# RKlompUU/fhe-regex

Measured on AMD Instinct MI355X. Metric: TFHE gate-bootstraps/sec; end-to-end match time for /abc/ on 256-char content, higher is better.
Workload: dtype u64

## Files before the change

### fhe-regex_amd/csrc/device.h

```cpp
#pragma once
#include <cstdint>
#include <vector>

#include "common.h"
#include "owned.h"

namespace fr {

constexpr int MAX_OUT = 8;
enum : int32_t { JOB_MULTI = 0, JOB_DIRECT = 1, JOB_SIGN = 2, JOB_ACC = 3 };
struct DevGate {
    int32_t n_in;
    int32_t offset;
    int32_t in_slot[16];
    int32_t in_w[16];
    int32_t n_out;
    int32_t direct;
    int32_t out_slot[MAX_OUT];
    uint8_t lut[MAX_OUT][16];
};
static_assert(sizeof(DevGate) == 304, "DevGate layout");
constexpr int MAX_SELECTORS = 2 * (int)NEEDLE_MAX_CHARS;
FR_HD uint32_t acc_selector(const DevGate& g) {
    return (uint32_t)g.lut[0][0] | ((uint32_t)g.lut[0][1] << 8) | ((uint32_t)g.lut[0][2] << 16) |
           ((uint32_t)g.lut[0][3] << 24);
}
inline void set_acc_selector(DevGate& g, uint32_t q) {
    for (int i = 0; i < 4; ++i) g.lut[0][i] = (uint8_t)(q >> (8 * i));
}
int lut_w_norm2(const uint8_t* lut);

struct DeviceTimers {
    double br_ms = 0, ks_ms = 0;
    uint64_t br_launches = 0, br_gates = 0, lut_outputs = 0;
    double lat_br_ms = 0;
    uint64_t lat_launches = 0, lat_gates = 0;
    double pair_br_ms = 0;
    uint64_t pair_launches = 0, pair_gates = 0;
};

struct ClientKey;
struct RngKey;
class Device;
using Slots = gpu::SlotsOf<Device>;

struct DevNeedle {
    gpu::DevBuf<uint64_t> words;
    size_t m = 0;
    Device* dev = nullptr;
    DevNeedle() = default;
    DevNeedle(DevNeedle&&) = default;
    DevNeedle& operator=(DevNeedle&&) = delete;
    ~DevNeedle();
};

class Device {
  public:
    Device(const Params& p, int device);
    ~Device();
    Device(const Device&) = delete;
    Device& operator=(const Device&) = delete;

    const Params& params() const { return p_; }
    int device() const { return dev_; }

    void upload_keys(const std::vector<uint64_t>& ksk, const std::vector<uint64_t>& bsk);
    bool has_keys() const { return ksk_ && (p_.ring == FR_RING_FFT ? bool(d_fbsk_[0]) : bool(d_bsk_)); }
    void gen_server_key(const ClientKey& ck, const RngKey& key, const RngKey* mask_key = nullptr);
    void load_server_key_compact(const RngKey& mask_key, const uint8_t* bodies);
    const double* key_load_ms() const { return key_load_ms_; }
    void download_server_key(uint64_t* ksk, size_t ksk_len, uint64_t* bsk, size_t bsk_len);
    void gen_packing_key(const ClientKey& ck, const RngKey& mask_key, const RngKey& noise_key, bool compact = false);
    void upload_packing_key(const void* rows);
    void download_packing_key(uint64_t* rows);
    void load_packing_key_compact(const RngKey& mask_key, const uint8_t* planes);
    void download_packing_key_compact(uint8_t* planes);
    const double* pk_load_ms() const { return pk_load_ms_; }
    bool has_packing_key() const { return bool(pksk_); }
    void packing_limb_column(int col, uint64_t* out_host);
    void pack_bools(const DevGate* gates, size_t n, uint64_t* out_host);
    void pack_bools_compact(const DevGate* gates, size_t n, uint16_t* out_host );
    const double* pack_ms() const { return pack_ms_; }
    void encrypt_to_slots(const ClientKey& ck, const uint8_t* msgs, size_t count, const RngKey& key, uint64_t first_block,
                          const int* slots);

    Slots expand_to_slots(const RngKey& mask_key, uint64_t first_block, const uint8_t* bodies, size_t count);
    double expand_ms() const { return expand_ms_; }

    int alloc_slot();
    void free_slot(int s);
    void write_slots(const int* slots, size_t n, const uint64_t* host );
    void read_slot(int slot, uint64_t* host );
    void slots_to_device(const int* slots, size_t n, uint64_t* dst);
    void device_to_slots(const int* slots, size_t n, const uint64_t* src);
    void slots_to_device_async(const int* slots, size_t n, uint64_t* dst);
    void* stream() const { return cur().stream.get(); }
    void zero_slot(int slot);
    size_t arena_slots() const { return next_slot_; }
    size_t arena_free_slots() const { return free_slots_.size(); }

    void run_level(const DevGate* gates, size_t n);
    void run_level_resident(const DevGate* d_gates, const DevGate* host, size_t n, size_t n_refs = 0);
    gpu::DevBuf<DevGate> upload_gates(const DevGate* gates, size_t n, size_t n_refs = 0);
    void bind_content(const int* cmap, size_t n);
    DevNeedle upload_needle(const uint64_t* words, size_t m);
    void bind_selectors(const uint64_t* table, size_t count);
    void run_linear(const DevGate& g);
    void sync();

    void set_lanes(int n);
    int match_lanes() const { return (int)lanes_.size(); }
    void enter_lane(int i);
    void leave_lane();
    void set_profiling(int level) { profiling_ = level; }
    DeviceTimers& timers() { return timers_; }

    void keyswitch_host(const uint64_t* in, size_t count, uint64_t* out);
    void blind_rotate_host(const uint64_t* ks_in, const uint8_t* luts, size_t count, uint64_t* out);
    void blind_rotate_multi_host(const uint64_t* ks_in, const uint8_t* luts, int n_out, int direct, uint64_t* out);
    void blind_rotate_acc_host(const uint64_t* ks_in, const uint64_t* accs, size_t count, uint64_t* out);
    void ring_mul_host(const uint64_t* a, const uint64_t* b, size_t count, uint64_t* out);
    void bench_pbs(const std::vector<DevGate>& gates, int iters, double* br_ms, double* total_ms);

    std::string info() const;

  private:
    struct LaneState {
        gpu::Stream stream;
        gpu::DevBuf<uint64_t> ks;
        gpu::DevBuf<int8_t> dig;
        gpu::DevBuf<DevGate> pk_gates;
        gpu::DevBuf<int8_t> pk_dig;
        gpu::DevBuf<uint64_t> pk_g;
        gpu::DevBuf<uint16_t> pk_c16;
        gpu::DevBuf<double> kpre;
        gpu::StagingRing<int> cmap;
        size_t cmap_n = 0;
        const uint64_t* sel = nullptr;
        size_t sel_n = 0;
        gpu::Event done_ev;
        bool pending = false;
    };
    LaneState lane0_;
    std::vector<LaneState> lanes_;
    int lane_ = 0;
    LaneState& cur() { return lane_ ? lanes_[lane_ - 1] : lane0_; }
    const LaneState& cur() const { return lane_ ? lanes_[lane_ - 1] : lane0_; }
    bool lanes_pending_ = false;
    bool lanes_unsynced_ = false;
    gpu::Event main_ev_;
    std::vector<int> deferred_free_;
    hipStream_t cur_stream();
    void join_lanes();
    void sync_all();
    void ensure_arena(size_t slots);
    void ensure_ks(size_t n);
    void ensure_gates(size_t n);
    void validate_gates(const DevGate* gates, size_t n, size_t n_refs = 0) const;
    void launch_level(const DevGate* d_gates, const DevGate* host, size_t n);
    gpu::Event take_event();
    void resolve_timers();
    void ensure_digits(size_t rows);
    struct LimbKey {
        gpu::DevBuf<uint64_t> rows;
        gpu::DevBuf<int8_t> limbs;
        int KD = 0, ncols = 0, nlc = 0;
        explicit operator bool() const { return rows && limbs; }
        void alloc_rows(int kd, int nc) {
            limbs.reset();
            KD = kd, ncols = nc, nlc = ((nc * 8 + 127) / 128) * 128;
            rows.alloc((size_t)kd * nc);
        }
        void reset() { rows.reset(), limbs.reset(); }
    };
    void build_limbs(LimbKey& key);
    void drop_server_key() {
        ksk_.reset(), d_tbsk_.reset(), d_bsk_.reset(), d_fbsk_[0].reset(), d_fbsk_[1].reset();
        lane0_.kpre.reset();
        for (auto& l : lanes_) l.kpre.reset();
    }
    void drop_packing_key() { pksk_.reset(); }
    struct KsShape {
        int MR;
        size_t padded;
        int MC = 1, GZ = 1;
        bool lds = true;
    };
    KsShape ks_shape(size_t n) const {
        const int MR = n >= ks_mr4_min_ ? 4 : 1;
        return {MR, (n + 32 * MR - 1) / (32 * MR) * (32 * MR)};
    }
    template <int KSB, int KSL>
    void launch_ks_digits(const DevGate* d_gates, size_t n, size_t padded, int8_t* dig, uint64_t* out, int out_n,
                          int out_stride, hipEvent_t ev_start);
    void launch_limb_gemm(const int8_t* dig, const LimbKey& key, size_t n, const KsShape& sh, uint64_t* out,
                          int out_stride, hipEvent_t ev_stop);
    void launch_ks(const DevGate* d_gates, size_t n, uint64_t* d_ks, hipEvent_t ev_start = nullptr,
                   hipEvent_t ev_stop = nullptr);
    void launch_br(const DevGate* d_gates, const uint64_t* d_ks, size_t n, hipEvent_t ev_start = nullptr,
                   hipEvent_t ev_stop = nullptr, bool acc = false);
    size_t leading_selector_jobs(const DevGate* host, size_t n) const;
    void launch_jobs(const DevGate* d_gates, const DevGate* host, size_t n, bool acc);
    void run_br_jobs(const uint64_t* ks_in, std::vector<DevGate>& gates, uint64_t* out);
    void init_rns();
    void upload_rns_bsk(const std::vector<uint64_t>& bsk);
    void launch_br_rns(const DevGate* d_gates, const uint64_t* d_ks, size_t n, hipEvent_t ev_start, hipEvent_t ev_stop);
    void init_ks();
    void init_fft();
    void upload_fft_bsk(const std::vector<uint64_t>& bsk);
    void launch_br_fft(const DevGate* d_gates, const uint64_t* d_ks, size_t n, hipStream_t stream,
                       hipEvent_t ev_start = nullptr, hipEvent_t ev_stop = nullptr, bool acc = false);
    void build_fourier_bsk();
    double key_load_ms_[5] = {0, 0, 0, 0, 0};
    double pk_load_ms_[3] = {0, 0, 0};
    gpu::StagingRing<uint8_t> xstage_;
    double expand_ms_ = 0;
    void stage_slot_list(const int* slots, size_t n);
    gpu::DevBuf<int> d_slot_list_;

    Params p_;
    int dev_;
    int e_ = 8;
    int e_small_ = 8;
    size_t small_batch_ = 256;
    LimbKey ksk_;
    gpu::DevBuf<uint64_t> d_tbsk_;
    LimbKey pksk_;
    double pack_ms_[4] = {0, 0, 0, 0};
    void pack_launch(const DevGate* gates, size_t n, uint64_t* out_words, uint16_t* out_c16);
    int pk_split_ = 0;
    bool ks_mfma_ = true;
    size_t ks_mr4_min_ = 96;
    int ks_mc_ = 0;
    int ks_split_ = 0;
    int ks_xcd_ = 1;
    bool ks_dig16_ = true;
    bool ks_lds_ = true;
    gpu::DevBuf<uint32_t> d_bsk_;
    gpu::DevBuf<uint32_t> d_tw_;
    int fft_e_ = 4;
    size_t fft_small_ = 256;
    size_t fft_pair_ = SIZE_MAX;
    bool fft_dual_ = false;
    size_t fft_kpre_ = 32;
    gpu::DevBuf<double> d_fbsk_[2];
    static int fbsk_index(int E) { return E == 4 ? 0 : 1; }
    bool fbsk_needed(int E) const { return E == 4 || E == fft_e_; }
    gpu::DevBuf<double> d_ftw_;
    gpu::DevBuf<double> d_fqt_;
    gpu::DevBuf<uint16_t> d_fleaf_;
    gpu::DevBuf<uint64_t> d_arena_;
    std::vector<int> free_slots_;
    size_t next_slot_ = 0;
    gpu::StagingRing<DevGate> gates_;
    struct PendingTimer {
        gpu::Event ev[4];
        size_t gates, outs;
        bool lat, pair, ks;
        bool chain;
    };
    bool latency_shape(size_t n) const;
    bool pair_shape(size_t n) const;
    std::vector<PendingTimer> pending_;
    std::vector<gpu::Event> event_pool_;
    int profiling_ = 0;
    bool timer_chain_ = true;
    DeviceTimers timers_;
    gpu::Event ev_[4];
};

}
```

### fhe-regex_amd/csrc/device.hip

```cpp
#include <algorithm>
#include <cstdlib>
#include <cstring>
#include <sstream>

#include "device_impl.h"

namespace fr {

static bool supported(const Params& p) {
    if (p.ring == FR_RING_FFT) return (p.N == 2048 && p.k == 1) || (p.N == 1024 && p.k == 2);
    return (p.N == 2048 && p.k == 1) || (p.N == 1024 && p.k == 2) || (p.N == 1024 && p.k == 1);
}

namespace gpu {
void* dev_alloc(size_t bytes) {
    void* p = nullptr;
    HIP_CHECK(hipMalloc(&p, bytes));
    return p;
}
void dev_free(void* p) noexcept { (void)hipFree(p); }
void* pinned_alloc(size_t bytes) {
    void* p = nullptr;
    HIP_CHECK(hipHostMalloc(&p, bytes));
    return p;
}
void pinned_free(void* p) noexcept { (void)hipHostFree(p); }
hipEvent_t event_create(unsigned flags) {
    hipEvent_t e = nullptr;
    HIP_CHECK(hipEventCreateWithFlags(&e, flags));
    return e;
}
void event_destroy(hipEvent_t e) noexcept { (void)hipEventDestroy(e); }
hipStream_t stream_create() {
    hipStream_t s = nullptr;
    HIP_CHECK(hipStreamCreateWithFlags(&s, hipStreamNonBlocking));
    return s;
}
void stream_destroy(hipStream_t s) noexcept { (void)hipStreamDestroy(s); }

void StagingBytes::reserve(size_t bytes, size_t first, hipStream_t s) {
    if (bytes <= d_.size()) return;
    size_t cap = d_.size() ? d_.size() : first;
    while (cap < bytes) cap *= 2;
    HIP_CHECK(hipStreamSynchronize(s));
    d_.reset();
    for (auto& h : h_) h.reset();
    try {
        for (auto& e : ev_)
            if (!e) e = Event(hipEventDisableTiming);
        for (auto& h : h_) h.alloc(cap);
        d_.alloc(cap);
    } catch (...) {
        for (auto& h : h_) h.reset();
        throw;
    }
}
void* StagingBytes::acquire() {
    side_ ^= 1;
    HIP_CHECK(hipEventSynchronize(ev_[side_].get()));
    return h_[side_].get();
}
void StagingBytes::commit(size_t bytes, hipStream_t s) {
    HIP_CHECK(hipMemcpyAsync(d_.get(), h_[side_].get(), bytes, hipMemcpyHostToDevice, s));
    HIP_CHECK(hipEventRecord(ev_[side_].get(), s));
}
}

Device::Device(const Params& p, int device) : p_(p), dev_(device) {
    if (!supported(p)) throw Error(FR_ERR_INVALID, "device: unsupported (k, N)");
    if (p.ks_base_log != 3 || p.ks_level != 5 || p.pbs_base_log != 23 || p.pbs_level != 1)
        throw Error(FR_ERR_INVALID, "device: only KS 2^3x5 and PBS 2^23x1 are compiled");
    if (p.n > 1024) throw Error(FR_ERR_INVALID, "device: n > 1024");
    int count = 0;
    if (hipGetDeviceCount(&count) != hipSuccess || count <= device || device < 0)
        throw Error(FR_ERR_NO_DEVICE, "no usable HIP device " + std::to_string(device));
    HIP_CHECK(hipSetDevice(device));
    lane0_.stream.create();
    for (auto& e : ev_) e = gpu::Event(hipEventDefault);
    init_rns();
    init_ks();
    if (const char* ev = std::getenv("FR_TIMER_CHAIN")) timer_chain_ = std::atoi(ev) != 0;
    if (p.ring == FR_RING_FFT) init_fft();
    ensure_arena(1024);
    ensure_ks(1024);
    ensure_gates(1024);
}

Device::~Device() {
    (void)hipSetDevice(dev_);
    for (auto& l : lanes_) (void)hipStreamSynchronize(l.stream.get());
    if (lane0_.stream) (void)hipStreamSynchronize(lane0_.stream.get());
}

void Device::set_lanes(int n) {
    if (n < 1 || n > 8) throw Error(FR_ERR_INVALID, "lanes: 1..8");
    if (lane_ != 0) throw Error(FR_ERR_INVALID, "lanes: changed inside a lane");
    sync_all();
    const int extra = n >= 2 ? n : 0;
    while ((int)lanes_.size() > extra) lanes_.pop_back();
    if (!main_ev_ && extra) main_ev_ = gpu::Event(hipEventDisableTiming);
    while ((int)lanes_.size() < extra) {
        LaneState l;
        l.stream.create();
        l.done_ev = gpu::Event(hipEventDisableTiming);
        lanes_.push_back(std::move(l));
        enter_lane((int)lanes_.size());
        ensure_ks(1024);
        leave_lane();
    }
}
void Device::enter_lane(int i) {
    if (lane_ != 0) throw Error(FR_ERR_INVALID, "lanes: already inside a lane");
    if (i <= 0) return;
    if (i > (int)lanes_.size()) throw Error(FR_ERR_INVALID, "lanes: no such lane");
    HIP_CHECK(hipEventRecord(main_ev_.get(), lane0_.stream.get()));
    HIP_CHECK(hipStreamWaitEvent(lanes_[i - 1].stream.get(), main_ev_.get(), 0));
    lane_ = i;
}
void Device::leave_lane() {
    if (lane_ == 0) return;
    LaneState& l = cur();
    HIP_CHECK(hipEventRecord(l.done_ev.get(), l.stream.get()));
    l.pending = true;
    lanes_pending_ = true;
    lanes_unsynced_ = true;
    lane_ = 0;
}
void Device::join_lanes() {
    if (!lanes_pending_ || lane_ != 0) return;
    for (auto& l : lanes_)
        if (l.pending) {
            HIP_CHECK(hipStreamWaitEvent(lane0_.stream.get(), l.done_ev.get(), 0));
            l.pending = false;
        }
    lanes_pending_ = false;
}
hipStream_t Device::cur_stream() {
    if (lane_ == 0 && lanes_pending_) join_lanes();
    return cur().stream.get();
}
void Device::sync_all() {
    HIP_CHECK(hipStreamSynchronize(lane0_.stream.get()));
    for (auto& l : lanes_) HIP_CHECK(hipStreamSynchronize(l.stream.get()));
    if (lane_ == 0) {
        for (auto& l : lanes_) l.pending = false;
        lanes_pending_ = false;
    }
    lanes_unsynced_ = false;
    free_slots_.insert(free_slots_.end(), deferred_free_.begin(), deferred_free_.end());
    deferred_free_.clear();
}

std::string Device::info() const {
    hipDeviceProp_t prop;
    (void)hipGetDeviceProperties(&prop, dev_);
    std::ostringstream o;
    o << prop.name << " " << prop.gcnArchName << " CUs=" << prop.multiProcessorCount;
    if (p_.ring == FR_RING_FFT) o << " ring=fft E=" << fft_e_ << " latency<=" << fft_small_;
    else o << " ring=rns E=" << e_;
    return o.str();
}

void Device::ensure_arena(size_t slots) {
    const size_t stride = p_.slot_stride(), have = d_arena_.size() / stride;
    if (slots <= have) return;
    size_t cap = have ? have : 1024;
    while (cap < slots) cap *= 2;
    gpu::DevBuf<uint64_t> nb(stride * cap);
    if (d_arena_) {
        sync_all();
        HIP_CHECK(hipMemcpyAsync(nb.get(), d_arena_.get(), 8 * d_arena_.size(), hipMemcpyDeviceToDevice, STREAM));
        HIP_CHECK(hipStreamSynchronize(STREAM));
    }
    d_arena_ = std::move(nb);
}

void Device::ensure_ks(size_t n) {
    const size_t row = p_.ks_stride();
    if (n * row <= cur().ks.size()) return;
    HIP_CHECK(hipStreamSynchronize(STREAM));
    cur().ks.grow(n * row, 1024 * row);
}
void Device::ensure_gates(size_t n) { gates_.reserve(n, 1024, STREAM); }

int Device::alloc_slot() {
    if (!free_slots_.empty()) {
        int s = free_slots_.back();
        free_slots_.pop_back();
        return s;
    }
    ensure_arena(next_slot_ + 1);
    return (int)next_slot_++;
}
void Device::free_slot(int s) {
    if (s < 0) return;
    if (lanes_unsynced_ || lane_ != 0) {
        deferred_free_.push_back(s);
        if (deferred_free_.size() >= (size_t)1 << 16) sync_all();
    } else {
        free_slots_.push_back(s);
    }
}

__global__ void __launch_bounds__(256) k_slots_to_buf(const uint64_t* __restrict__ arena, int stride,
                                                      const int* __restrict__ slots, int len, uint64_t* __restrict__ buf) {
    const uint64_t* s = arena + (size_t)slots[blockIdx.x] * stride;
    uint64_t* d = buf + (size_t)blockIdx.x * len;
    for (int c = threadIdx.x; c < len; c += 256) d[c] = s[c];
}
__global__ void __launch_bounds__(256) k_buf_to_slots(const uint64_t* __restrict__ buf, int len,
                                                      const int* __restrict__ slots, int stride, uint64_t* __restrict__ arena) {
    const uint64_t* s = buf + (size_t)blockIdx.x * len;
    uint64_t* d = arena + (size_t)slots[blockIdx.x] * stride;
    for (int c = threadIdx.x; c < len; c += 256) d[c] = s[c];
}
struct SlotArgs {
    int s[16];
};
__global__ void __launch_bounds__(256) k_slots_to_buf_arg(const uint64_t* __restrict__ arena, int stride, SlotArgs sl,
                                                          int len, uint64_t* __restrict__ buf) {
    const uint64_t* s = arena + (size_t)sl.s[blockIdx.x] * stride;
    uint64_t* d = buf + (size_t)blockIdx.x * len;
    for (int c = threadIdx.x; c < len; c += 256) d[c] = s[c];
}
void Device::slots_to_device_async(const int* slots, size_t n, uint64_t* dst) {
    if (!n) return;
    if (n > 16) throw Error(FR_ERR_INVALID, "slots_to_device_async: at most 16 slots");
    SlotArgs a{};
    for (size_t i = 0; i < n; ++i) {
        if (slots[i] < 0 || (size_t)slots[i] >= next_slot_) throw Error(FR_ERR_INVALID, "slot list: slot out of range");
        a.s[i] = slots[i];
    }
    k_slots_to_buf_arg<<<(unsigned)n, 256, 0, STREAM>>>(d_arena_.get(), p_.slot_stride(), a, p_.lwe_len(), dst);
    HIP_CHECK(hipGetLastError());
}
void Device::stage_slot_list(const int* slots, size_t n) {
    for (size_t i = 0; i < n; ++i)
        if (slots[i] < 0 || (size_t)slots[i] >= next_slot_) throw Error(FR_ERR_INVALID, "slot list: slot out of range");
    if (n > d_slot_list_.size()) {
        HIP_CHECK(hipStreamSynchronize(STREAM));
        d_slot_list_.alloc(std::max<size_t>(n, 1024));
    }
    HIP_CHECK(hipMemcpyAsync(d_slot_list_.get(), slots, 4 * n, hipMemcpyHostToDevice, STREAM));
}
void Device::slots_to_device(const int* slots, size_t n, uint64_t* dst) {
    if (!n) return;
    stage_slot_list(slots, n);
    k_slots_to_buf<<<(unsigned)n, 256, 0, STREAM>>>(d_arena_.get(), p_.slot_stride(), d_slot_list_.get(), p_.lwe_len(), dst);
    HIP_CHECK(hipGetLastError());
    HIP_CHECK(hipStreamSynchronize(STREAM));
}
void Device::device_to_slots(const int* slots, size_t n, const uint64_t* src) {
    if (!n) return;
    stage_slot_list(slots, n);
    k_buf_to_slots<<<(unsigned)n, 256, 0, STREAM>>>(src, p_.lwe_len(), d_slot_list_.get(), p_.slot_stride(), d_arena_.get());
    HIP_CHECK(hipGetLastError());
    HIP_CHECK(hipStreamSynchronize(STREAM));
}

void Device::write_slots(const int* slots, size_t n, const uint64_t* host) {
    const int L = p_.lwe_len(), S = p_.slot_stride();
    for (size_t i = 0; i < n; ++i)
        HIP_CHECK(hipMemcpyAsync(d_arena_.get() + (size_t)slots[i] * S, host + i * L, 8 * (size_t)L, hipMemcpyHostToDevice, STREAM));
    HIP_CHECK(hipStreamSynchronize(STREAM));
}
void Device::read_slot(int slot, uint64_t* host) {
    HIP_CHECK(hipMemcpyAsync(host, d_arena_.get() + (size_t)slot * p_.slot_stride(), 8 * (size_t)p_.lwe_len(),
                             hipMemcpyDeviceToHost, STREAM));
    sync_all();
}
void Device::zero_slot(int slot) {
    HIP_CHECK(hipMemsetAsync(d_arena_.get() + (size_t)slot * p_.slot_stride(), 0, 8 * (size_t)p_.lwe_len(), STREAM));
}

void Device::upload_keys(const std::vector<uint64_t>& ksk, const std::vector<uint64_t>& bsk) {
    if (ksk.size() != (size_t)p_.big() * p_.ks_level * (p_.n + 1)) throw Error(FR_ERR_INVALID, "ksk size");
    if (bsk.size() != p_.bsk_len()) throw Error(FR_ERR_INVALID, "bsk size");
    Replacing key_guard([this] { drop_server_key(); });
    ksk_.alloc_rows(p_.big() * p_.ks_level, p_.n + 1);
    HIP_CHECK(hipMemcpy(ksk_.rows.get(), ksk.data(), 8 * ksk.size(), hipMemcpyHostToDevice));
    build_limbs(ksk_);
    if (p_.ring == FR_RING_FFT) upload_fft_bsk(bsk);
    else upload_rns_bsk(bsk);
    key_guard.dismiss();
}

bool Device::latency_shape(size_t n) const { return n <= (p_.ring == FR_RING_FFT ? fft_small_ : small_batch_); }
bool Device::pair_shape(size_t n) const { return p_.ring == FR_RING_FFT && !latency_shape(n) && n <= fft_pair_; }

void Device::launch_br(const DevGate* d_gates, const uint64_t* d_ks, size_t n, hipEvent_t ev_start, hipEvent_t ev_stop,
                       bool acc) {
    if (acc && p_.ring != FR_RING_FFT) throw Error(FR_ERR_INVALID, "private search: FFT ring only");
    if (p_.ring == FR_RING_FFT) launch_br_fft(d_gates, d_ks, n, cur().stream.get(), ev_start, ev_stop, acc);
    else launch_br_rns(d_gates, d_ks, n, ev_start, ev_stop);
}

void Device::validate_gates(const DevGate* gates, size_t n, size_t n_refs) const {
    for (size_t i = 0; i < n; ++i) {
        const DevGate& g = gates[i];
        if (g.n_in < 0 || g.n_in > 16 || g.n_out < 1 || g.n_out > MAX_OUT || g.direct < 0 || g.direct > JOB_ACC ||
            (g.direct && g.n_out != 1))
            throw Error(FR_ERR_INVALID, "device gate: bad descriptor");
        if (g.direct == JOB_ACC) {
            if (p_.ring != FR_RING_FFT) throw Error(FR_ERR_INVALID, "private search: FFT ring only");
            if (acc_selector(g) >= (uint32_t)MAX_SELECTORS) throw Error(FR_ERR_INVALID, "device gate: bad selector index");
        }
        for (int f = 0; f < g.n_out; ++f)
            if (g.out_slot[f] < 0 || (size_t)g.out_slot[f] >= next_slot_) throw Error(FR_ERR_INVALID, "device gate: bad output slot");
        for (int q = 0; q < g.n_in; ++q) {
            const int s = g.in_slot[q];
            if (s >= 0 ? (size_t)s >= next_slot_ : (size_t)(-1 - (int64_t)s) >= n_refs)
                throw Error(FR_ERR_INVALID, "device gate: bad input slot");
        }
    }
}

void Device::bind_content(const int* cmap, size_t n) {
    for (size_t i = 0; i < n; ++i)
        if (cmap[i] < -1 || (cmap[i] >= 0 && (size_t)cmap[i] >= next_slot_))
            throw Error(FR_ERR_INVALID, "content map: slot out of range");
    LaneState& l = cur();
    const size_t bound = l.cmap_n;
    l.cmap_n = 0;
    if (!n) return;
    const hipStream_t s = STREAM;
    l.cmap.reserve(n, 4096, s);
    if (n != bound || std::memcmp(l.cmap.last(), cmap, 4 * n) != 0) {
        std::memcpy(l.cmap.acquire(), cmap, 4 * n);
        l.cmap.commit(n, s);
    }
    l.cmap_n = n;
}

DevNeedle::~DevNeedle() {
    if (!words || !dev) return;
    try {
        dev->sync();
    } catch (...) {
    }
}

DevNeedle Device::upload_needle(const uint64_t* words, size_t m) {
    if (p_.ring != FR_RING_FFT) throw Error(FR_ERR_INVALID, "private search: FFT ring only");
    if (!words || m < 1 || 2 * m > (size_t)MAX_SELECTORS) throw Error(FR_ERR_INVALID, "needle: 1 <= m <= 64");
    DevNeedle nd;
    nd.dev = this;
    nd.m = m;
    nd.words.alloc(2 * m * (size_t)(p_.k + 1) * p_.N);
    HIP_CHECK(hipMemcpy(nd.words.get(), words, 8 * nd.words.size(), hipMemcpyHostToDevice));
    return nd;
}

void Device::bind_selectors(const uint64_t* table, size_t count) {
    if (table && p_.ring != FR_RING_FFT) throw Error(FR_ERR_INVALID, "private search: FFT ring only");
    cur().sel = table;
    cur().sel_n = table ? count : 0;
}

size_t Device::leading_selector_jobs(const DevGate* host, size_t n) const {
    if (!n || host[0].direct != JOB_ACC) return 0;
    size_t a = 0;
    while (a < n && host[a].direct == JOB_ACC) ++a;
    for (size_t i = 0; i < n; ++i) {
        if (host[i].direct != JOB_ACC) continue;
        if (i >= a) throw Error(FR_ERR_INVALID, "selector jobs must lead their level");
        if ((size_t)acc_selector(host[i]) >= cur().sel_n)
            throw Error(FR_ERR_INVALID, "selector job: index past the selector table bound");
    }
    return a;
}

void Device::run_level(const DevGate* gates, size_t n) {
    if (!n) return;
    if (!has_keys()) throw Error(FR_ERR_NO_KEY, "server key not uploaded");
    if (lane_ != 0) throw Error(FR_ERR_INVALID, "staged gate batches run on lane 0 only");
    validate_gates(gates, n);
    ensure_ks(n);
    ensure_gates(n);
    std::memcpy(gates_.acquire(), gates, sizeof(DevGate) * n);
    gates_.commit(n, STREAM);
    launch_level(gates_.device(), gates, n);
}

void Device::run_level_resident(const DevGate* d_gates, const DevGate* host, size_t n, size_t n_refs) {
    if (!n) return;
    if (!has_keys()) throw Error(FR_ERR_NO_KEY, "server key not uploaded");
    if (n_refs > cur().cmap_n) throw Error(FR_ERR_INVALID, "template plan: content map not bound");
    ensure_ks(n);
    launch_level(d_gates, host, n);
}

gpu::DevBuf<DevGate> Device::upload_gates(const DevGate* gates, size_t n, size_t n_refs) {
    validate_gates(gates, n, n_refs);
    gpu::DevBuf<DevGate> d(std::max<size_t>(n, 1));
    HIP_CHECK(hipMemcpy(d.get(), gates, sizeof(DevGate) * n, hipMemcpyHostToDevice));
    return d;
}

void Device::launch_level(const DevGate* d_gates, const DevGate* host, size_t n) {
    const size_t a = leading_selector_jobs(host, n);
    if (a) launch_jobs(d_gates, host, a, true);
    if (n > a) launch_jobs(d_gates + a, host + a, n - a, false);
}

void Device::launch_jobs(const DevGate* d_gates, const DevGate* host, size_t n, bool acc) {
    PendingTimer t{};
    if (profiling_)
        for (auto& e : t.ev) e = take_event();
    t.chain = profiling_ == 1 && timer_chain_;
    uint64_t* d_ks = cur().ks.get();
    if (profiling_ >= 2) launch_ks(d_gates, n, d_ks, t.ev[0].get(), t.ev[1].get());
    else launch_ks(d_gates, n, d_ks, nullptr, t.chain ? t.ev[1].get() : nullptr);
    launch_br(d_gates, d_ks, n, t.chain ? nullptr : t.ev[2].get(), t.ev[3].get(), acc);
    HIP_CHECK(hipGetLastError());
    if (profiling_) {
        t.gates = n;
        t.lat = latency_shape(n);
        t.pair = pair_shape(n) && (!fft_dual_ || acc);
        t.ks = profiling_ >= 2;
        t.outs = 0;
        for (size_t i = 0; i < n; ++i) t.outs += host[i].n_out;
        pending_.push_back(std::move(t));
    }
}

gpu::Event Device::take_event() {
    if (!event_pool_.empty()) {
        gpu::Event e = std::move(event_pool_.back());
        event_pool_.pop_back();
        return e;
    }
    for (unsigned fl : {(unsigned)hipEventReleaseToDevice, (unsigned)hipEventDisableSystemFence})
        try {
            return gpu::Event(fl);
        } catch (const Error&) {
            (void)hipGetLastError();
        }
    return gpu::Event(hipEventDefault);
}
void Device::resolve_timers() {
    for (auto& t : pending_) {
        float ks = 0, br = 0;
        if (t.ks) HIP_CHECK(hipEventElapsedTime(&ks, t.ev[0].get(), t.ev[1].get()));
        HIP_CHECK(hipEventElapsedTime(&br, t.ev[t.chain ? 1 : 2].get(), t.ev[3].get()));
        timers_.ks_ms += ks;
        timers_.br_ms += br;
        timers_.br_launches += 1;
        timers_.br_gates += t.gates;
        timers_.lut_outputs += t.outs;
        if (t.lat) {
            timers_.lat_br_ms += br;
            timers_.lat_launches += 1;
            timers_.lat_gates += t.gates;
        }
        if (t.pair) {
            timers_.pair_br_ms += br;
            timers_.pair_launches += 1;
            timers_.pair_gates += t.gates;
        }
        for (auto& e : t.ev)
            if (e) event_pool_.push_back(std::move(e));
    }
    pending_.clear();
}

void Device::sync() {
    sync_all();
    resolve_timers();
}

void Device::keyswitch_host(const uint64_t* in, size_t count, uint64_t* out) {
    if (!has_keys()) throw Error(FR_ERR_NO_KEY, "server key not uploaded");
    HIP_CHECK(hipStreamSynchronize(STREAM));
    Slots slots(*this, count);
    std::vector<DevGate> gates(count);
    write_slots(slots.data(), count, in);
    for (size_t i = 0; i < count; ++i) {
        std::memset(&gates[i], 0, sizeof(DevGate));
        gates[i].n_in = 1;
        gates[i].in_slot[0] = slots[i];
        gates[i].in_w[0] = 1;
        gates[i].n_out = 1;
        gates[i].direct = JOB_DIRECT;
        gates[i].out_slot[0] = slots[i];
    }
    ensure_ks(count);
    ensure_gates(count);
    uint64_t* d_ks = cur().ks.get();
    HIP_CHECK(hipMemcpy(gates_.device(), gates.data(), sizeof(DevGate) * count, hipMemcpyHostToDevice));
    launch_ks(gates_.device(), count, d_ks);
    HIP_CHECK(hipStreamSynchronize(STREAM));
    const int ks = p_.ks_stride();
    for (size_t i = 0; i < count; ++i)
        HIP_CHECK(hipMemcpy(out + i * (p_.n + 1), d_ks + i * ks, 8 * (size_t)(p_.n + 1), hipMemcpyDeviceToHost));
}

static DevGate br_job(const uint8_t* luts, int n_out, int direct) {
    DevGate g;
    std::memset(&g, 0, sizeof g);
    g.n_out = n_out;
    g.direct = direct;
    std::memcpy(g.lut, luts, 16 * (size_t)n_out);
    return g;
}

void Device::run_br_jobs(const uint64_t* ks_in, std::vector<DevGate>& gates, uint64_t* out) {
    if (!has_keys()) throw Error(FR_ERR_NO_KEY, "server key not uploaded");
    HIP_CHECK(hipStreamSynchronize(STREAM));
    const size_t count = gates.size();
    ensure_ks(count);
    ensure_gates(count);
    uint64_t* d_ks = cur().ks.get();
    const int ks = p_.ks_stride();
    for (size_t i = 0; i < count; ++i)
        HIP_CHECK(hipMemcpy(d_ks + i * ks, ks_in + i * (p_.n + 1), 8 * (size_t)(p_.n + 1), hipMemcpyHostToDevice));
    size_t n_out = 0;
    for (auto& g : gates) n_out += (size_t)g.n_out;
    Slots slots(*this, n_out);
    n_out = 0;
    for (auto& g : gates)
        for (int f = 0; f < g.n_out; ++f) g.out_slot[f] = slots[n_out++];
    HIP_CHECK(hipMemcpy(gates_.device(), gates.data(), sizeof(DevGate) * count, hipMemcpyHostToDevice));
    const size_t a = leading_selector_jobs(gates.data(), count);
    if (a && a != count) throw Error(FR_ERR_INVALID, "a launch is all selector jobs or none");
    PendingTimer t{};
    if (profiling_) {
        t.ev[2] = take_event(), t.ev[3] = take_event();
        t.gates = count, t.outs = n_out;
        t.lat = latency_shape(count);
        t.pair = pair_shape(count) && (!fft_dual_ || a != 0);
    }
    launch_br(gates_.device(), d_ks, count, t.ev[2].get(), t.ev[3].get(), a != 0);
    if (profiling_) {
        pending_.push_back(std::move(t));
        sync();
    } else {
        HIP_CHECK(hipStreamSynchronize(STREAM));
    }
    for (size_t i = 0; i < slots.size(); ++i) read_slot(slots[i], out + i * p_.lwe_len());
}

void Device::blind_rotate_acc_host(const uint64_t* ks_in, const uint64_t* accs, size_t count, uint64_t* out) {
    if (p_.ring != FR_RING_FFT) throw Error(FR_ERR_INVALID, "private search: FFT ring only");
    if (!has_keys()) throw Error(FR_ERR_NO_KEY, "server key not uploaded");
    if (lane_ != 0) throw Error(FR_ERR_INVALID, "parity hooks run on lane 0 only");
    if (!count) return;
    const size_t W = (size_t)(p_.k + 1) * p_.N;
    gpu::DevBuf<uint64_t> table(count * W);
    HIP_CHECK(hipMemcpy(table.get(), accs, 8 * count * W, hipMemcpyHostToDevice));
    std::vector<DevGate> gates(count);
    for (size_t i = 0; i < count; ++i) {
        std::memset(&gates[i], 0, sizeof(DevGate));
        gates[i].n_out = 1;
        gates[i].direct = JOB_ACC;
        set_acc_selector(gates[i], (uint32_t)i);
    }
    const uint64_t* prev = cur().sel;
    const size_t prev_n = cur().sel_n;
    bind_selectors(table.get(), count);
    try {
        run_br_jobs(ks_in, gates, out);
    } catch (...) {
        (void)hipStreamSynchronize(cur().stream.get());
        bind_selectors(prev, prev_n);
        throw;
    }
    bind_selectors(prev, prev_n);
}

void Device::blind_rotate_host(const uint64_t* ks_in, const uint8_t* luts, size_t count, uint64_t* out) {
    std::vector<DevGate> gates(count);
    for (size_t i = 0; i < count; ++i) gates[i] = br_job(luts + 16 * i, 1, JOB_DIRECT);
    run_br_jobs(ks_in, gates, out);
}

void Device::blind_rotate_multi_host(const uint64_t* ks_in, const uint8_t* luts, int n_out, int direct,
                                     uint64_t* out) {
    if (!has_keys()) throw Error(FR_ERR_NO_KEY, "server key not uploaded");
    if (n_out < 1 || n_out > MAX_OUT || direct < 0 || direct > 2 || (direct && n_out != 1))
        throw Error(FR_ERR_INVALID, "bad n_out");
    std::vector<DevGate> gates{br_job(luts, n_out, direct)};
    run_br_jobs(ks_in, gates, out);
}

int lut_w_norm2(const uint8_t* lut) {
    int s = 0;
    for (int m = 1; m < 16; ++m) s += ((int)lut[m] - lut[m - 1]) * ((int)lut[m] - lut[m - 1]);
    s += ((int)lut[0] + lut[15]) * ((int)lut[0] + lut[15]);
    return s;
}

void Device::bench_pbs(const std::vector<DevGate>& gates, int iters, double* br_ms, double* total_ms) {
    const size_t n = gates.size();
    ensure_ks(n);
    ensure_gates(n);
    sync();
    std::memcpy(gates_.acquire(), gates.data(), sizeof(DevGate) * n);
    gates_.commit(n, STREAM);
    const DevGate* d_gates = gates_.device();
    uint64_t* d_ks = cur().ks.get();
    float br_sum = 0;
    HIP_CHECK(hipEventRecord(ev_[3].get(), STREAM));
    for (int it = 0; it < iters; ++it) {
        launch_ks(d_gates, n, d_ks);
        HIP_CHECK(hipEventRecord(ev_[1].get(), STREAM));
        launch_br(d_gates, d_ks, n);
        HIP_CHECK(hipEventRecord(ev_[2].get(), STREAM));
        HIP_CHECK(hipEventSynchronize(ev_[2].get()));
        float br = 0;
        HIP_CHECK(hipEventElapsedTime(&br, ev_[1].get(), ev_[2].get()));
        br_sum += br;
    }
    HIP_CHECK(hipEventRecord(ev_[0].get(), STREAM));
    HIP_CHECK(hipEventSynchronize(ev_[0].get()));
    float tot = 0;
    HIP_CHECK(hipEventElapsedTime(&tot, ev_[3].get(), ev_[0].get()));
    *br_ms = br_sum;
    *total_ms = tot;
}

}
```

### fhe-regex_amd/csrc/fft_br.hip

```cpp
#include <hip/hip_ext.h>
#include <hip/hip_runtime.h>

#include <cstring>

#include "device_impl.h"
#include "fft.h"
#include "geo.h"

namespace fr {

template <int M, int E>
using FGeo = NttGeo<M, E, 3, fft_layout_variant(ilog2c(M), ilog2c(E))>;
template <int M, int E>
constexpr int FV = fft_layout_variant(ilog2c(M), ilog2c(E));

__device__ __forceinline__ void cfwd(double2& x, double2& y, double2 c) { fft::fwd_bf(x.x, x.y, y.x, y.y, c.x, c.y); }
__device__ __forceinline__ void cinv(double2& u, double2& v, double2 c) { fft::inv_bf(u.x, u.y, v.x, v.y, c.x, c.y); }

template <int M, int E>
constexpr bool fradix4() {
    return E == 4 && FGeo<M, E>::LOG % 2 == 0;
}
template <int M, int E>
struct FTwr {
    static constexpr int COUNT = fradix4<M, E>() ? FGeo<M, E>::NPH * 3 : FGeo<M, E>::LOG * (E / 2);
    double2 v[COUNT];
};
__device__ __forceinline__ double2 fmul_i(double2 c) { return make_double2(-c.y, c.x); }
__device__ __forceinline__ void cinv_r4(double2 (&x)[4], double2 c, double2 ca, double2 cc) {
    fft::inv_r4(x[0].x, x[0].y, x[1].x, x[1].y, x[2].x, x[2].y, x[3].x, x[3].y, c.x, c.y, ca.x, ca.y, cc.x, cc.y);
}
template <class G, int E, int p, bool REV, class F>
__device__ __forceinline__ void for_butterflies(F&& fn) {
#pragma unroll
    for (int i = 0; i < G::s_end(p) - G::s_begin(p); ++i) {
        const int s = REV ? G::s_end(p) - 1 - i : G::s_begin(p) + i;
        const int dm = 1 << (G::LOG - 1 - s - G::lo(p));
#pragma unroll
        for (int m = 0; m < E; ++m) {
            if (m & dm) continue;
            fn(s, m, dm);
        }
    }
}
template <class G, int p>
__device__ __forceinline__ double2 ftw_at(const double2* tw, int b, int s, int m) {
    return (tw + (b >> (G::LOG - s)))[(1 << s) + (G::template moff<p>(m) >> (G::LOG - s))];
}
template <int M, int E, int p>
__device__ __forceinline__ void ftw_r4(const double2* tw, int tl, double2& c, double2& ca) {
    using G = FGeo<M, E>;
    constexpr int s0 = G::s_begin(p), s1 = s0 + 1;
    const int b = G::template base<p>(tl);
    c = ftw_at<G, p>(tw, b, s0, 0);
    ca = ftw_at<G, p>(tw, b, s1, 0);
}

template <int M, int E, int p>
__device__ __forceinline__ void ffwd_phase(double2 (&x)[E], const double2* tw, int tl) {
    using G = FGeo<M, E>;
    const int b = G::template base<p>(tl);
    for_butterflies<G, E, p, false>([&](int s, int m, int dm) { cfwd(x[m], x[m + dm], ftw_at<G, p>(tw, b, s, m)); });
}
template <int M, int E, int p>
__device__ __forceinline__ void finv_phase(double2 (&x)[E], const double2* tw, int tl) {
    using G = FGeo<M, E>;
    const int b = G::template base<p>(tl);
    for_butterflies<G, E, p, true>([&](int s, int m, int dm) { cinv(x[m], x[m + dm], ftw_at<G, p>(tw, b, s, m)); });
}
template <int M, int E, int p>
__device__ __forceinline__ void finv_phase_lds(double2 (&x)[E], const double2* tw, const double2* twc, int tl) {
    if constexpr (fradix4<M, E>()) {
        using G = FGeo<M, E>;
        double2 c, ca;
        ftw_r4<M, E, p>(tw, tl, c, ca);
        const double2 cc = ftw_at<G, p>(twc, G::template base<p>(tl), G::s_begin(p), 0);
        cinv_r4(x, c, ca, cc);
    } else {
        finv_phase<M, E, p>(x, tw, tl);
    }
}

#ifndef FR_LAT_LOAD1
#define FR_LAT_LOAD1 2
#endif
#ifndef FR_LAT_LOAD2
#define FR_LAT_LOAD2 3
#endif
#ifndef FR_LAT_PF
#define FR_LAT_PF 2
#endif
#ifndef FR_LAT_PF2
#define FR_LAT_PF2 2
#endif
#ifndef FR_PAIR_LOAD
#define FR_PAIR_LOAD 2
#endif
#ifndef FR_PAIR_PF
#define FR_PAIR_PF 1
#endif
#ifndef FR_PAIR_LOAD2
#define FR_PAIR_LOAD2 4
#endif
#ifndef FR_PAIR_CC
#define FR_PAIR_CC 1
#endif
#ifndef FR_LAT_TWR
#define FR_LAT_TWR 1
#endif

template <int M, int E, int p>
constexpr bool ftw_wave_uniform() {
    using G = FGeo<M, E>;
    for (int w = 0; w * 64 < G::T; ++w)
        for (int s = G::s_begin(p); s < G::s_end(p); ++s) {
            const int ref = geo_base(G::LOG, G::e, p, w * 64, FV<M, E>) >> (G::LOG - s);
            for (int l = 1; l < 64; ++l)
                if ((geo_base(G::LOG, G::e, p, w * 64 + l, FV<M, E>) >> (G::LOG - s)) != ref) return false;
        }
    return true;
}
__device__ __forceinline__ double2 fwave_uniform(double2 v) {
    const unsigned long long a = (unsigned long long)__double_as_longlong(v.x);
    const unsigned long long b = (unsigned long long)__double_as_longlong(v.y);
    const unsigned a0 = __builtin_amdgcn_readfirstlane((unsigned)a), a1 = __builtin_amdgcn_readfirstlane((unsigned)(a >> 32));
    const unsigned b0 = __builtin_amdgcn_readfirstlane((unsigned)b), b1 = __builtin_amdgcn_readfirstlane((unsigned)(b >> 32));
    return make_double2(__longlong_as_double((long long)(((unsigned long long)a1 << 32) | a0)),
                        __longlong_as_double((long long)(((unsigned long long)b1 << 32) | b0)));
}
#ifndef FR_TW_SGPR_PAIR
#define FR_TW_SGPR_PAIR 1
#endif

template <int M, int E>
constexpr int ftw_index(int s, int m) {
    const int d = FGeo<M, E>::LOG - 1 - s - FGeo<M, E>::lo(s / FGeo<M, E>::e);
    return s * (E / 2) + ((m >> (d + 1)) << d) + (m & ((1 << d) - 1));
}
template <int M, int E, int p, bool UNI = false>
__device__ __forceinline__ void ftw_load_phase(FTwr<M, E>& twr, const double2* tw, int tl) {
    using G = FGeo<M, E>;
    if constexpr (fradix4<M, E>()) {
        double2 c, ca, cc;
        ftw_r4<M, E, p>(tw, tl, c, ca);
        fft::cmul(c.x, c.y, ca.x, ca.y, cc.x, cc.y);
        if constexpr (UNI && ftw_wave_uniform<M, E, p>()) {
            c = fwave_uniform(c);
            ca = fwave_uniform(ca);
            cc = fwave_uniform(cc);
        }
        twr.v[3 * p] = c, twr.v[3 * p + 1] = ca, twr.v[3 * p + 2] = cc;
        if constexpr (p + 1 < G::NPH) ftw_load_phase<M, E, p + 1, UNI>(twr, tw, tl);
        return;
    }
    const int b = G::template base<p>(tl);
    for_butterflies<G, E, p, false>([&](int s, int m, int) { twr.v[ftw_index<M, E>(s, m)] = ftw_at<G, p>(tw, b, s, m); });
    if constexpr (p + 1 < G::NPH) ftw_load_phase<M, E, p + 1, UNI>(twr, tw, tl);
}
template <int M, int E, int p>
__device__ __forceinline__ void ffwd_phase_r(double2 (&x)[E], const FTwr<M, E>& twr) {
    using G = FGeo<M, E>;
    if constexpr (fradix4<M, E>()) {
        const double2 c = twr.v[3 * p], ca = twr.v[3 * p + 1];
        cfwd(x[0], x[2], c);
        cfwd(x[1], x[3], c);
        cfwd(x[0], x[1], ca);
        cfwd(x[2], x[3], fmul_i(ca));
        return;
    }
    for_butterflies<G, E, p, false>([&](int s, int m, int dm) { cfwd(x[m], x[m + dm], twr.v[ftw_index<M, E>(s, m)]); });
}
template <int M, int E, int p>
__device__ __forceinline__ void finv_phase_r(double2 (&x)[E], const FTwr<M, E>& twr) {
    using G = FGeo<M, E>;
    if constexpr (fradix4<M, E>()) {
        cinv_r4(x, twr.v[3 * p], twr.v[3 * p + 1], twr.v[3 * p + 2]);
        return;
    }
    for_butterflies<G, E, p, true>([&](int s, int m, int dm) { cinv(x[m], x[m + dm], twr.v[ftw_index<M, E>(s, m)]); });
}

template <int M, int E, int PF, int PT>
constexpr int fperm_lane_bit(int j) {
    using G = FGeo<M, E>;
    const int out = G::lo(PF) + j, in = G::lo(PT) + j;
    int kb = -1, kc = -1;
    for (int b = 0; b < 6; ++b) {
        if (G::lane_bit(PT, b) == out) kb = b;
        if (G::lane_bit(PF, b) == in) kc = b;
    }
    return kb == kc ? kb : -1;
}
template <int M, int E, int PF, int PT>
constexpr bool fperm_ok() {
    using G = FGeo<M, E>;
    if (PF == PT || (PF - PT != 1 && PT - PF != 1)) return false;
    for (int j = 0; j < G::e; ++j) {
        const int k = fperm_lane_bit<M, E, PF, PT>(j);
        if (k != 4 && k != 5) return false;
    }
    for (int b = 0; b < 8; ++b) {
        bool swapped = false;
        for (int j = 0; j < G::e; ++j) swapped |= fperm_lane_bit<M, E, PF, PT>(j) == b;
        if (!swapped && G::lane_bit(PF, b) != G::lane_bit(PT, b)) return false;
    }
    return true;
}
template <int K>
__device__ __forceinline__ void fperm_swap(double& a, double& b) {
    static_assert(K == 4 || K == 5, "permlane swaps serve lane bits 4 and 5");
    const unsigned long long ua = (unsigned long long)__double_as_longlong(a);
    const unsigned long long ub = (unsigned long long)__double_as_longlong(b);
    unsigned lo0 = (unsigned)ua, hi0 = (unsigned)(ua >> 32), lo1 = (unsigned)ub, hi1 = (unsigned)(ub >> 32);
    if constexpr (K == 4) {
        const auto l = __builtin_amdgcn_permlane16_swap(lo0, lo1, false, false);
        const auto h = __builtin_amdgcn_permlane16_swap(hi0, hi1, false, false);
        lo0 = l[0], lo1 = l[1], hi0 = h[0], hi1 = h[1];
    } else {
        const auto l = __builtin_amdgcn_permlane32_swap(lo0, lo1, false, false);
        const auto h = __builtin_amdgcn_permlane32_swap(hi0, hi1, false, false);
        lo0 = l[0], lo1 = l[1], hi0 = h[0], hi1 = h[1];
    }
    a = __longlong_as_double((long long)(((unsigned long long)hi0 << 32) | lo0));
    b = __longlong_as_double((long long)(((unsigned long long)hi1 << 32) | lo1));
}
template <int M, int E, int PF, int PT, int j = 0>
__device__ __forceinline__ void fperm_exchange(double2 (&x)[E]) {
    constexpr int K = fperm_lane_bit<M, E, PF, PT>(j);
#pragma unroll
    for (int m = 0; m < E; ++m) {
        if (m & (1 << j)) continue;
        fperm_swap<K>(x[m].x, x[m | (1 << j)].x);
        fperm_swap<K>(x[m].y, x[m | (1 << j)].y);
    }
    if constexpr (j + 1 < FGeo<M, E>::e) fperm_exchange<M, E, PF, PT, j + 1>(x);
}

#ifndef FR_XKEEP
#define FR_XKEEP 1
#endif
template <int M, int E, int PF, int PT>
constexpr bool fxkeep_ok() {
    using G = FGeo<M, E>;
    if (!FR_XKEEP || (1 << (6 + G::e)) > G::T || PF == PT) return false;
    for (int b = 0; (1 << b) < G::T; ++b) {
        if (b >= 6 && b < 6 + G::e) {
            if (G::lane_bit(PF, b) != G::lo(PT) + (b - 6) || G::lane_bit(PT, b) != G::lo(PF) + (b - 6)) return false;
        } else if (G::lane_bit(PF, b) != G::lane_bit(PT, b)) {
            return false;
        }
    }
    return true;
}
template <int M, int E, int PF, int PT, bool PRE, bool XK, int B, int BS>
__device__ __forceinline__ void fexchange(double2 (&x)[B][E], double2* row, int tl) {
    using G = FGeo<M, E>;
    if constexpr (fperm_ok<M, E, PF, PT>()) {
        static_assert(!PRE, "register exchanges replace only exchanges without a pre-barrier");
#pragma unroll
        for (int b = 0; b < B; ++b) fperm_exchange<M, E, PF, PT>(x[b]);
    } else {
        constexpr int X = PF < PT ? PF : PT;
        double2* rf = row + G::template at<X>(G::template base<PF>(tl));
        double2* rt = row + G::template at<X>(G::template base<PT>(tl));
        if constexpr (PRE) __syncthreads();
        if constexpr (XK && fxkeep_ok<M, E, PF, PT>()) {
            const int q = __builtin_amdgcn_readfirstlane((tl >> 6) & (E - 1));
#pragma unroll
            for (int b = 0; b < B; ++b)
#pragma unroll
                for (int m = 0; m < E; ++m)
                    if (m != q) rf[b * BS + G::template at<X>(G::template moff<PF>(m))] = x[b][m];
            __syncthreads();
#pragma unroll
            for (int b = 0; b < B; ++b)
#pragma unroll
                for (int m = 0; m < E; ++m)
                    if (m != q) x[b][m] = rt[b * BS + G::template at<X>(G::template moff<PT>(m))];
            return;
        }
#pragma unroll
        for (int b = 0; b < B; ++b)
#pragma unroll
            for (int m = 0; m < E; ++m) rf[b * BS + G::template at<X>(G::template moff<PF>(m))] = x[b][m];
        if constexpr (G::template wave_local<PF, PT>() && G::wave_top(PF)) wave_sync();
        else __syncthreads();
#pragma unroll
        for (int b = 0; b < B; ++b)
#pragma unroll
            for (int m = 0; m < E; ++m) x[b][m] = rt[b * BS + G::template at<X>(G::template moff<PT>(m))];
    }
}
template <int M, int E, int X = 0>
constexpr bool fexchanges_conflict_free() {
    using G = FGeo<M, E>;
    if constexpr (X + 1 >= G::NPH) return true;
    else
        return ((fperm_ok<M, E, X, X + 1>() && X != G::XL) || G::template b128_exchange_ok<X>()) &&
               fexchanges_conflict_free<M, E, X + 1>();
}
template <int M, int E, int p, bool NOPRE, bool TWR, int B, int BS, bool CARRY = false, class Hook>
__device__ __forceinline__ void fforward_from(double2 (&x)[B][E], double2* row, const FTwr<M, TWR ? E : 2>& twr,
                                              const double2* tw, int tl, Hook&& hook) {
#pragma unroll
    for (int b = 0; b < B; ++b) {
        if constexpr (TWR) ffwd_phase_r<M, E, p>(x[b], twr);
        else ffwd_phase<M, E, p>(x[b], tw, tl);
    }
    hook(std::integral_constant<int, p>{});
    if constexpr (p + 1 < FGeo<M, E>::NPH) {
        constexpr bool pre = !NOPRE && (FGeo<M, E>::template fwd_pre<p>() || CARRY), reg = fperm_ok<M, E, p, p + 1>();
        fexchange<M, E, p, p + 1, reg ? false : pre, !NOPRE, B, BS>(x, row, tl);
        fforward_from<M, E, p + 1, NOPRE, TWR, B, BS, reg && pre>(x, row, twr, tw, tl, hook);
    }
}
template <int M, int E, int p, bool NOPRE, bool TWR, int B, int BS, bool CARRY = false>
__device__ __forceinline__ void finverse_from(double2 (&x)[B][E], double2* row, const FTwr<M, TWR ? E : 2>& twr,
                                              const double2* tw, const double2* twc, int tl) {
    if constexpr (TWR && B > 1 && fradix4<M, E>() && FR_PAIR_CC) {
        const double2 c = twr.v[3 * p], ca = twr.v[3 * p + 1];
        double2 cc;
        fft::cmul(c.x, c.y, ca.x, ca.y, cc.x, cc.y);
#pragma unroll
        for (int b = 0; b < B; ++b) cinv_r4(x[b], c, ca, cc);
    } else {
#pragma unroll
        for (int b = 0; b < B; ++b) {
            if constexpr (TWR) finv_phase_r<M, E, p>(x[b], twr);
            else finv_phase_lds<M, E, p>(x[b], tw, twc, tl);
        }
    }
    if constexpr (p > 0) {
        constexpr bool pre = !NOPRE && (FGeo<M, E>::template inv_pre<p>() || CARRY), reg = fperm_ok<M, E, p, p - 1>();
        fexchange<M, E, p, p - 1, reg ? false : pre, !NOPRE, B, BS>(x, row, tl);
        finverse_from<M, E, p - 1, NOPRE, TWR, B, BS, reg && pre>(x, row, twr, tw, twc, tl);
    }
}

template <int N, int K, int E>
constexpr int fbr_threads() {
    return (K + 1) * (N / 2 / E);
}
__device__ __forceinline__ int psi_slot(int k) { return k ^ ((k >> 6) & 15) ^ ((k >> 5) & 1); }

__device__ __forceinline__ void slot_factor(double br, double bi, uint32_t e, uint32_t sm, double& cr, double& ci) {
    const uint32_t q = (e * sm) & 3u;
    const bool swap = (sm & 1u) && (e & 1u);
    const double ar = swap ? -bi : br, ai = swap ? br : bi;
    const long long sg = (long long)((q >> 1) & 1u) << 63;
    cr = __longlong_as_double(__double_as_longlong(ar) ^ sg);
    ci = __longlong_as_double(__double_as_longlong(ai) ^ sg);
}
template <int N, bool PSIQ>
__device__ __forceinline__ void key_psi_base(const double2* psi, uint32_t e, uint32_t Lb, double& br, double& bi) {
    const uint32_t k = __umul24(e, Lb) & (2 * N - 1);
    if constexpr (!PSIQ) {
        const double2 c = psi[psi_slot((int)k)];
        br = c.x;
        bi = c.y;
    } else {
        const double2 q = psi[psi_slot((int)(k & (N / 2 - 1)))];
        fft::psi_quadrant(q.x, q.y, k >> (ilog2c(N) - 1), br, bi);
    }
}
template <int K, int NB, class KeyAt>
__device__ __forceinline__ void key_products(const double (&bre)[2][NB], const double (&bim)[2][NB], int mb, uint32_t ei,
                                             uint32_t ej, uint32_t sm, KeyAt&& key, double& kor, double& koi,
                                             double (&kxr)[K], double (&kxi)[K]) {
    double cr[3], ci[3];
#pragma unroll
    for (int h = 1; h < 3; ++h)
        slot_factor(bre[h - 1][mb], bim[h - 1][mb], h == 1 ? ei : ej, sm, cr[h], ci[h]);
    fft::cmul(cr[1], ci[1], cr[2], ci[2], cr[0], ci[0]);
#pragma unroll
    for (int gg = 0; gg < 3; ++gg) {
        const double c1r = cr[gg] - 1.0, c1i = ci[gg];
        const double2 Bo = key(gg, 0);
        if (gg == 0) fft::cmul(Bo.x, Bo.y, c1r, c1i, kor, koi);
        else fft::cmac(Bo.x, Bo.y, c1r, c1i, kor, koi);
#pragma unroll
        for (int q = 0; q < K; ++q) {
            const double2 Bx = key(gg, 1 + q);
            if (gg == 0) fft::cmul(Bx.x, Bx.y, c1r, c1i, kxr[q], kxi[q]);
            else fft::cmac(Bx.x, Bx.y, c1r, c1i, kxr[q], kxi[q]);
        }
    }
}
template <int K, bool LAT>
constexpr bool fbr_twr() {
    return LAT && K == 1 && FR_LAT_TWR;
}
template <int N, int K, int E, bool LAT>
constexpr int fbr_twc_entries() {
    return fradix4<N / 2, E>() && !fbr_twr<K, LAT>() ? N / 4 : 0;
}
template <int N, int K, int E, bool LAT, int B = 1, bool KP = false>
constexpr size_t fbr_smem_bytes() {
    return 16 * ((LAT ? 2 : 1) * B * (K + 1) * (size_t)FGeo<N / 2, E>::NP + (B == 1 ? (size_t)N / 2 : 0) +
                 (KP ? 0 : LAT && B == 1 ? 2 * (size_t)N : (size_t)N / 2) + (size_t)fbr_twc_entries<N, K, E, LAT>()) +
           B * (16 * MAX_OUT + 2 * 1026) + (B == 1 ? 4 * 17 * MAX_OUT : 0) + 2 * 514;
}
template <int K, int E>
constexpr int fbr_tp_groups() {
    return K == 1 ? 2 : (E == 8 ? 3 : 2);
}
template <int N, int K, int E, bool LAT>
constexpr int fbr_min_waves() {
    if (LAT) return 2;
    if (K == 1) return E == 4 ? 4 : 2;
    return E == 4 ? 3 : 2;
}
typedef unsigned int fr_v4u __attribute__((ext_vector_type(4)));
__device__ __forceinline__ __amdgpu_buffer_rsrc_t bsk_rsrc(const double2* bsk) {
    return __builtin_amdgcn_make_buffer_rsrc((void*)bsk, 0, 0x7fffffff, 0x00020000);
}
__device__ __forceinline__ double2 bsk_load(__amdgpu_buffer_rsrc_t r, uint32_t lane_off, uint32_t uoff) {
    const fr_v4u v = __builtin_amdgcn_raw_buffer_load_b128(r, (int)lane_off, (int)uoff, 0);
    double2 d;
    __builtin_memcpy(&d, &v, 16);
    return d;
}

template <int K>
__device__ __forceinline__ int other_row(int P, int q) {
    return q < P ? q : q + 1;
}
template <int M, int T, int K>
__device__ __forceinline__ void load_slot(double2 (&B)[3][K + 1], __amdgpu_buffer_rsrc_t rs, uint32_t sbase, int P,
                                          int m, uint32_t lane_off) {
    constexpr uint32_t GG = (uint32_t)(K + 1) * (K + 1) * M;
#pragma unroll
    for (int gg = 0; gg < 3; ++gg) {
        B[gg][0] = bsk_load(rs, lane_off, sbase + 16u * (gg * GG + (uint32_t)(P * (K + 1) + P) * M + (uint32_t)m * T));
#pragma unroll
        for (int q = 0; q < K; ++q)
            B[gg][1 + q] = bsk_load(
                rs, lane_off, sbase + 16u * (gg * GG + (uint32_t)(other_row<K>(P, q) * (K + 1) + P) * M + (uint32_t)m * T));
    }
}

template <int N>
__device__ __forceinline__ uint64_t test_poly(int t, bool direct, const uint8_t* lut0) {
    constexpr int box = N / 16, half = box / 2;
    if (!direct) return 1ULL << (DELTA_LOG - 1);
    const int mm = (t + half) / box;
    return mm < 16 ? (uint64_t)lut0[mm] << DELTA_LOG : (uint64_t)0 - ((uint64_t)lut0[0] << DELTA_LOG);
}
template <int N>
__device__ __forceinline__ uint64_t w_step64(const uint64_t* row, const uint32_t* terms, int nt, int j) {
    uint64_t acc = 0;
    for (int t = 0; t < nt; ++t) {
        const uint32_t tm = terms[t];
        int src = j - (int)(tm & 0xFFFF);
        int64_t d = (int64_t)(tm >> 16) - 128;
        if (src < 0) {
            src += N;
            d = -d;
        }
        acc += (uint64_t)d * row[src];
    }
    return acc;
}

template <int M, int E>
__device__ __forceinline__ void fbr_publish(uint64_t* arow, const double (&alo)[E], const double (&ahi)[E], int tl) {
#pragma unroll
    for (int m = 0; m < E; ++m) {
        const int j = FGeo<M, E>::template idx<0>(tl, m);
        arow[j] = fft::torus_of_acc(alo[m]);
        arow[j + M] = fft::torus_of_acc(ahi[m]);
    }
}
template <int N>
__device__ __forceinline__ void fbr_terms(int tid, int n_out, int kind, const uint8_t* lut, uint32_t* wterms, int* wcnt) {
    if (tid < n_out && kind == JOB_MULTI) wcnt[tid] = lut_terms<N>(lut + 16 * tid, wterms + 16 * tid);
}
template <int N, int K, int NT>
__device__ __forceinline__ void fbr_outputs(int tid, const uint64_t* ab, const DevGate& gate, int n_out, int kind,
                                            const uint32_t* wterms, const int* wcnt, uint64_t* arena, int slot_stride) {
    constexpr int big = K * N;
    if (kind != JOB_MULTI) {
        uint64_t* out = arena + (size_t)gate.out_slot[0] * slot_stride;
        const uint64_t post = kind == JOB_SIGN ? (1ULL << (DELTA_LOG - 1)) : 0;
        for (int c = tid; c <= big; c += NT) {
            const ExtractIdx x = extract_index<N, K>(c);
            const uint64_t v = ab[x.pp * N + x.j];
            out[c] = (x.neg ? (uint64_t)0 - v : v) + (c == big ? post : 0);
        }
        return;
    }
    for (int f = 0; f < n_out; ++f) {
        const uint32_t* tf = wterms + 16 * f;
        const int nt = wcnt[f];
        uint64_t* out = arena + (size_t)gate.out_slot[f] * slot_stride;
        for (int c = tid; c <= big; c += NT) {
            const ExtractIdx x = extract_index<N, K>(c);
            const uint64_t v = w_step64<N>(ab + x.pp * N, tf, nt, x.j);
            out[c] = x.neg ? (uint64_t)0 - v : v;
        }
    }
}

template <int N, int K>
constexpr uint32_t kpre_step_bytes() {
    return 16u * (uint32_t)((K + 1) * (K + 1) * (N / 2));
}

template <int N, int K, int E, bool LAT, int B, bool KP, bool ACC = false>
__device__ __forceinline__ void fbr_rotate(const uint64_t* ks, int ks_stride, int n, const DevGate* gates, int n_gates,
                                           const double2* bsk, const double2* tw_g, const double2* psi_g,
                                           const uint16_t* leaf_g, uint64_t* arena, int slot_stride, const double2* kpre,
                                           const uint64_t* sel = nullptr) {
    constexpr int M = N / 2;
    static_assert(!KP || (LAT && B == 1 && K == 1 && E == 4), "key products: the k = 1 latency shape");
    static_assert(!(ACC && KP), "selector launches never take the key-products path");
    using G = FGeo<M, E>;
    static_assert(fexchanges_conflict_free<M, E>(), "LDS maps must make every exchange conflict-free");
    static_assert(G::base_matches_geo(), "base<p> must be the index map the LDS-map proofs reason about");
    static_assert(G::key_slot_matches_idx(), "the Fourier key's lane layout is the last-phase layout");
    static_assert(!LAT || E == 4, "the latency shape holds a step's GGSW values in registers: E = 4");
    static_assert(B == 1 || (B == 2 && LAT && K == 1 && E == 4), "pair shape: the k = 1 latency geometry");
    constexpr int NB = E >= 4 ? E / 4 : 1;
    constexpr int T = M / E, NT = (K + 1) * T, LAST = G::NPH - 1, XL = G::XL;
    constexpr int LOG2N2 = G::LOG + 2;
    constexpr bool TWR = fbr_twr<K, LAT>();
    constexpr int BS = (K + 1) * G::NP;
    constexpr bool PSIQ = !LAT || B > 1;
    extern __shared__ __attribute__((aligned(16))) double2 fsm[];
    double2* xbuf = fsm;
    double2* ibuf = LAT ? xbuf + B * BS : xbuf;
    double2* tw = xbuf + (LAT ? 2 : 1) * B * BS;
    constexpr int NPSI = KP ? 0 : PSIQ ? N / 2 : 2 * N;
    double2* psi = tw + (B == 1 ? M : 0);
    double2* twc = psi + NPSI;
    constexpr int NTWC = fbr_twc_entries<N, K, E, LAT>();
    uint8_t* lut = (uint8_t*)(twc + NTWC);
    uint16_t* abar = (uint16_t*)(lut + B * 16 * MAX_OUT);
    uint32_t* wterms = B == 1 ? (uint32_t*)(abar + 1026) : (uint32_t*)ibuf;
    int* wcnt = (int*)(wterms + B * 16 * MAX_OUT);
    uint16_t* nxt = B == 1 ? (uint16_t*)(wcnt + MAX_OUT) : abar + B * 1026;

    const int tid = threadIdx.x;
    const int P = __builtin_amdgcn_readfirstlane(tid / T), tl = tid % T;
    int gb[B];
    bool has[B];
    const uint64_t* in[B];
    int n_out[B], kind[B];
#pragma unroll
    for (int b = 0; b < B; ++b) {
        const int gi = B * (int)blockIdx.x + b;
        has[b] = gi < n_gates;
        gb[b] = has[b] ? gi : B * (int)blockIdx.x;
        in[b] = ks + (size_t)gb[b] * ks_stride;
        n_out[b] = gates[gb[b]].n_out;
        kind[b] = gates[gb[b]].direct;
    }
    if constexpr (B == 1)
        for (int i = tid; i < M; i += NT) tw[i] = tw_g[i];
    for (int i = tid; i < NPSI; i += NT) psi[psi_slot(i)] = psi_g[i];
    for (int i = 1 + tid; i < NTWC; i += NT) {
        const int s0 = 31 - __builtin_clz((unsigned)i), b = i - (1 << s0);
        if (s0 & 1) continue;
        const double2 c = tw_g[i], ca = tw_g[(2 << s0) + 2 * b];
        fft::cmul(c.x, c.y, ca.x, ca.y, twc[i].x, twc[i].y);
    }
    uint32_t bbar[B];
#pragma unroll
    for (int b = 0; b < B; ++b) {
        uint8_t* lb = lut + b * 16 * MAX_OUT;
        uint16_t* ab = abar + b * 1026;
        for (int i = tid; i < 16 * n_out[b]; i += NT) lb[i] = gates[gb[b]].lut[i / 16][i % 16];
        for (int i = tid; i < n; i += NT) ab[i] = (uint16_t)mod_switch(in[b][i], LOG2N2);
        if (tid == 0) ab[n] = 0;
        bbar[b] = mod_switch(in[b][n], LOG2N2);
    }
    uint32_t Lb[NB];
#pragma unroll
    for (int bb = 0; bb < NB; ++bb)
        Lb[bb] = (1u + 4u * (__brev((uint32_t)G::template idx<LAST>(tl, 4 * bb)) >> (32 - G::LOG))) & (uint32_t)(M - 1);
    __syncthreads();

    double alo[B][E], ahi[B][E];
#pragma unroll
    for (int b = 0; b < B; ++b) {
        if constexpr (ACC) {
            const uint64_t* A = sel + ((size_t)acc_selector(gates[gb[b]]) * (K + 1) + P) * N;
#pragma unroll
            for (int m = 0; m < E; ++m) {
                const int j = G::template idx<0>(tl, m);
                uint64_t v[2];
#pragma unroll
                for (int h = 0; h < 2; ++h) {
                    const int s = (j + h * M + (int)bbar[b]) & (2 * N - 1);
                    const uint64_t tv = A[s & (N - 1)];
                    v[h] = s < N ? tv : (uint64_t)0 - tv;
                }
                alo[b][m] = fft::acc_of_torus(v[0]);
                ahi[b][m] = fft::acc_of_torus(v[1]);
            }
            continue;
        }
        const bool direct = kind[b] == JOB_DIRECT;
#pragma unroll
        for (int m = 0; m < E; ++m) {
            const int j = G::template idx<0>(tl, m);
            uint64_t v[2];
#pragma unroll
            for (int h = 0; h < 2; ++h) {
                const int s = (j + h * M + (int)bbar[b]) & (2 * N - 1);
                const uint64_t tv = test_poly<N>(s & (N - 1), direct, lut + b * 16 * MAX_OUT);
                v[h] = s < N ? tv : (uint64_t)0 - tv;
            }
            alo[b][m] = P == K ? fft::acc_of_torus(v[0]) : 0.0;
            ahi[b][m] = P == K ? fft::acc_of_torus(v[1]) : 0.0;
        }
    }

    double2* row = xbuf + P * G::NP;
    double2* irow = ibuf + P * G::NP;
    const int bl = G::template base<LAST>(tl);
    double2* row_bl = row + G::template at<XL>(bl);
    const double2* orow_bl[K];
#pragma unroll
    for (int q = 0; q < K; ++q) orow_bl[q] = xbuf + other_row<K>(P, q) * G::NP + G::template at<XL>(bl);
    constexpr uint32_t GG = (uint32_t)(K + 1) * (K + 1) * M;
    const __amdgpu_buffer_rsrc_t rs = bsk_rsrc(bsk);
    const uint32_t lane_off = 16u * (uint32_t)tl;
    const int steps = (n + 1) / 2;
    double2 gv[3][K + 1][LAT && !KP ? E : 1];
    double2 kv[K + 1][KP ? E : 1];
    FTwr<M, TWR ? E : 2> twr;
    if constexpr (TWR) ftw_load_phase<M, E, 0, B == 1 ? false : FR_TW_SGPR_PAIR>(twr, B == 1 ? tw : tw_g, tl);
#ifdef FR_BR_TIMING
    uint64_t tseg[6] = {0, 0, 0, 0, 0, 0};
    uint64_t tlast = __builtin_amdgcn_s_memtime();
    const uint64_t tstart = tlast;
#endif
    auto load_ggsw = [&](int gg, int tt) {
        if constexpr (!KP) {
            const uint32_t sb = (uint32_t)__builtin_amdgcn_readfirstlane(tt) * (3u * GG * 16u);
#pragma unroll
            for (int m = 0; m < E; ++m) {
                gv[gg][0][m] =
                    bsk_load(rs, lane_off, sb + 16u * (gg * GG + (uint32_t)(P * (K + 1) + P) * M + (uint32_t)m * T));
#pragma unroll
                for (int q = 0; q < K; ++q)
                    gv[gg][1 + q][m] = bsk_load(
                        rs, lane_off,
                        sb + 16u * (gg * GG + (uint32_t)(other_row<K>(P, q) * (K + 1) + P) * M + (uint32_t)m * T));
            }
        }
    };
    const __amdgpu_buffer_rsrc_t rk =
        bsk_rsrc(KP ? kpre + (size_t)blockIdx.x * ((size_t)((n + 1) / 2) * (kpre_step_bytes<N, K>() / 16)) : bsk);
    auto load_kp = [&](int tt) {
        if constexpr (KP) {
            const uint32_t sb = (uint32_t)__builtin_amdgcn_readfirstlane(tt) * kpre_step_bytes<N, K>();
#pragma unroll
            for (int r = 0; r <= K; ++r)
#pragma unroll
                for (int m = 0; m < E; ++m)
                    kv[r][m] = bsk_load(rk, lane_off, sb + 16u * (uint32_t)(((P * (K + 1) + r) * E + m) * T));
        }
    };
    constexpr int NPF = KP ? 0 : LAT ? (B > 1 ? FR_PAIR_PF : K == 1 ? FR_LAT_PF : FR_LAT_PF2) : 0;
    constexpr bool LATPF = NPF > 0;
    auto idle = [&](int t) {
        uint32_t z = 0;
#pragma unroll
        for (int b = 0; b < B; ++b) z |= abar[b * 1026 + 2 * t] | abar[b * 1026 + 2 * t + 1];
        return z == 0;
    };
    if constexpr (LATPF || KP) {
        for (int t = tid; t <= steps; t += NT) {
            int tt = t;
            while (tt < steps && idle(tt)) ++tt;
            nxt[t] = (uint16_t)tt;
        }
        __syncthreads();
        const int t0 = __builtin_amdgcn_readfirstlane((int)nxt[0]);
        for (int gg = 0; gg < NPF; ++gg) load_ggsw(gg, t0 < steps ? t0 : 0);
        load_kp(t0 < steps ? t0 : 0);
    }
    for (int t = 0; t < steps; ++t) {
        if (idle(t)) continue;
        BR_STAMP(0);
        const uint32_t sbase = (uint32_t)__builtin_amdgcn_readfirstlane(t) * (3u * GG * 16u);
        constexpr int G_TOP = !LAT || KP || B > 1 ? 3 : (NPF < 2 || K == 1) ? NPF : 3;
        constexpr int G_L1 = !LAT || KP ? 3 : B > 1 ? NPF : G_TOP + 1 < 3 ? G_TOP + 1 : 3;
        constexpr int G_L2 = !LAT || KP ? 3 : B > 1 ? (NPF + 1 < 3 ? NPF + 1 : 3) : G_TOP == 3 ? NPF : G_TOP + 2 < 3 ? G_TOP + 2 : 3;
        constexpr int PH_L1 = B > 1 ? FR_PAIR_LOAD : FR_LAT_LOAD1;
        constexpr int PH_L2 = B > 1 ? FR_PAIR_LOAD2 : FR_LAT_LOAD2;
        static_assert(G_L1 >= 3 || PH_L1 < G::NPH, "FR_PAIR_LOAD / FR_LAT_LOAD1 past the last forward phase");
        static_assert(G_L2 >= 3 || PH_L2 < G::NPH, "FR_PAIR_LOAD2 / FR_LAT_LOAD2 past the last forward phase");
        if constexpr (G_TOP < 3) {
            __builtin_amdgcn_sched_barrier(0);
            load_ggsw(G_TOP, t);
            __builtin_amdgcn_sched_barrier(0);
        }
        uint32_t ei[B], ej[B];
#pragma unroll
        for (int b = 0; b < B; ++b) {
            ei[b] = __builtin_amdgcn_readfirstlane((uint32_t)abar[b * 1026 + 2 * t]);
            ej[b] = __builtin_amdgcn_readfirstlane((uint32_t)abar[b * 1026 + 2 * t + 1]);
        }
        double bre[B][2][NB], bim[B][2][NB];
        auto psi_factors = [&]() {
#pragma unroll
            for (int b = 0; b < B; ++b)
#pragma unroll
                for (int h = 0; h < 2; ++h)
#pragma unroll
                    for (int bb = 0; bb < NB; ++bb)
                        key_psi_base<N, PSIQ>(psi, h == 0 ? ei[b] : ej[b], Lb[bb], bre[b][h][bb], bim[b][h][bb]);
        };
        if constexpr (LAT && B == 1 && !KP) psi_factors();
        double2 x[B][E];
#pragma unroll
        for (int b = 0; b < B; ++b)
#pragma unroll
            for (int m = 0; m < E; ++m)
                x[b][m] = make_double2(fft::acc_digit<23>(alo[b][m]), fft::acc_digit<23>(ahi[b][m]));
        BR_STAMP(1);
        fforward_from<M, E, 0, LAT, TWR, B, BS>(x, row, twr, tw, tl, [&](auto ph) {
            if constexpr (LAT) {
                constexpr int p = decltype(ph)::value;
                if constexpr (p == PH_L1 && G_L1 < 3) {
                    __builtin_amdgcn_sched_barrier(0);
                    load_ggsw(G_L1, t);
                    __builtin_amdgcn_sched_barrier(0);
                }
                if constexpr (p == PH_L2 && G_L2 < 3) {
                    __builtin_amdgcn_sched_barrier(0);
                    load_ggsw(G_L2, t);
                    __builtin_amdgcn_sched_barrier(0);
                }
            }
        });
        BR_STAMP(2);
#pragma unroll
        for (int b = 0; b < B; ++b)
#pragma unroll
            for (int m = 0; m < E; ++m) row_bl[b * BS + G::template at<XL>(G::template moff<LAST>(m))] = x[b][m];
        constexpr bool AHEAD = !LAT && E == 8;
        constexpr bool PRE0 = !LAT;
        double2 Bc[3][K + 1];
        if constexpr (PRE0) load_slot<M, T, K>(Bc, rs, sbase, P, 0, lane_off);
        __syncthreads();
        if constexpr (!LAT || B > 1) psi_factors();
#pragma unroll
        for (int m = 0; m < E; ++m) {
            double2 Bn[3][K + 1];
            if constexpr (AHEAD) {
                if (m + 1 < E) load_slot<M, T, K>(Bn, rs, sbase, P, m + 1, lane_off);
                __builtin_amdgcn_sched_barrier(0);
            } else if constexpr (!LAT) {
                if (!PRE0 || m > 0) load_slot<M, T, K>(Bc, rs, sbase, P, m, lane_off);
            }
#pragma unroll
            for (int b = 0; b < B; ++b) {
                const double2 own = x[b][m];
                double2 oth[K];
#pragma unroll
                for (int q = 0; q < K; ++q) oth[q] = orow_bl[q][b * BS + G::template at<XL>(G::template moff<LAST>(m))];
                double kor, koi, kxr[K], kxi[K];
                if constexpr (KP) {
                    kor = kv[0][m].x, koi = kv[0][m].y;
#pragma unroll
                    for (int q = 0; q < K; ++q) kxr[q] = kv[1 + q][m].x, kxi[q] = kv[1 + q][m].y;
                } else {
                    const uint32_t sm = ((m & 1) << 1) | ((m >> 1) & 1);
                    auto key_at = [&](int gg, int r) __attribute__((always_inline)) {
                        return LAT ? gv[gg][r][LAT ? m : 0] : Bc[gg][r];
                    };
                    key_products<K>(bre[b], bim[b], m >> 2, ei[b], ej[b], sm, key_at, kor, koi, kxr, kxi);
                }
                double zr, zi;
                fft::cmul(own.x, own.y, kor, koi, zr, zi);
#pragma unroll
                for (int q = 0; q < K; ++q) fft::cmac(oth[q].x, oth[q].y, kxr[q], kxi[q], zr, zi);
                x[b][m] = make_double2(zr, zi);
            }
            if constexpr (!LAT) {
                __builtin_amdgcn_sched_barrier(0);
            }
            if constexpr (AHEAD) {
#pragma unroll
                for (int gg = 0; gg < 3; ++gg)
#pragma unroll
                    for (int r = 0; r <= K; ++r) Bc[gg][r] = Bn[gg][r];
            }
        }
        if constexpr (LATPF || KP) {
            const int tn = __builtin_amdgcn_readfirstlane((int)nxt[t + 1]);
            __builtin_amdgcn_sched_barrier(0);
            for (int gg = 0; gg < NPF; ++gg) load_ggsw(gg, tn < steps ? tn : t);
            load_kp(tn < steps ? tn : t);
            __builtin_amdgcn_sched_barrier(0);
        }
        BR_STAMP(3);
        finverse_from<M, E, LAST, LAT, TWR, B, BS>(x, irow, twr, tw, twc, tl);
        BR_STAMP(4);
#pragma unroll
        for (int b = 0; b < B; ++b)
#pragma unroll
            for (int m = 0; m < E; ++m) {
                alo[b][m] = fft::acc_reduce<23>(alo[b][m] + x[b][m].x);
                ahi[b][m] = fft::acc_reduce<23>(ahi[b][m] + x[b][m].y);
            }
        BR_STAMP(5);
    }
#ifdef FR_BR_TIMING
    if (blockIdx.x == 0 && tid == 0)
        printf("FBR_TIMING E=%d LAT=%d steps=%d total=%lu digits=%lu fwd=%lu mac=%lu inv=%lu acc=%lu top=%lu\n", E, (int)LAT,
               steps, (unsigned long)(__builtin_amdgcn_s_memtime() - tstart), (unsigned long)tseg[1],
               (unsigned long)tseg[2], (unsigned long)tseg[3], (unsigned long)tseg[4], (unsigned long)tseg[5],
               (unsigned long)tseg[0]);
#endif

    __syncthreads();
    uint64_t* accs = (uint64_t*)xbuf;
    static_assert(B == 1 || 8 * B * (K + 1) * N <= 16 * B * BS, "pair shape: u64 rows inside the forward rows");
#pragma unroll
    for (int b = 0; b < B; ++b) {
        fbr_publish<M, E>(accs + (b * (K + 1) + P) * N, alo[b], ahi[b], tl);
        fbr_terms<N>(tid, n_out[b], kind[b], lut + b * 16 * MAX_OUT, wterms + b * 16 * MAX_OUT, wcnt + b * MAX_OUT);
    }
    __syncthreads();
#pragma unroll
    for (int b = 0; b < B; ++b)
        if (has[b])
            fbr_outputs<N, K, NT>(tid, accs + b * (K + 1) * N, gates[gb[b]], n_out[b], kind[b], wterms + b * 16 * MAX_OUT,
                                  wcnt + b * MAX_OUT, arena, slot_stride);
}

template <int N, int K, int E, bool LAT, int B = 1>
__global__ void __launch_bounds__((fbr_threads<N, K, E>()), (fbr_min_waves<N, K, E, LAT>()))
k_blind_rotate_fft(const uint64_t* __restrict__ ks, int ks_stride, int n, const DevGate* __restrict__ gates,
                   int n_gates, const double2* __restrict__ bsk, const double2* __restrict__ tw_g,
                   const double2* __restrict__ psi_g, const uint16_t* __restrict__ leaf_g, uint64_t* __restrict__ arena,
                   int slot_stride) {
    fbr_rotate<N, K, E, LAT, B, false>(ks, ks_stride, n, gates, n_gates, bsk, tw_g, psi_g, leaf_g, arena, slot_stride,
                                       nullptr);
}
template <int N, int K, int E, bool LAT, int B = 1>
__global__ void __launch_bounds__((fbr_threads<N, K, E>()), (fbr_min_waves<N, K, E, LAT>()))
k_blind_rotate_fft_kp(const uint64_t* __restrict__ ks, int ks_stride, int n, const DevGate* __restrict__ gates,
                      int n_gates, const double2* __restrict__ tw_g, uint64_t* __restrict__ arena, int slot_stride,
                      const double2* __restrict__ kpre) {
    fbr_rotate<N, K, E, LAT, B, true>(ks, ks_stride, n, gates, n_gates, nullptr, tw_g, nullptr, nullptr, arena,
                                      slot_stride, kpre);
}

template <int N, int K, int E, bool LAT, int B = 1>
__global__ void __launch_bounds__((fbr_threads<N, K, E>()), (fbr_min_waves<N, K, E, LAT>()))
k_blind_rotate_fft_acc(const uint64_t* __restrict__ ks, int ks_stride, int n, const DevGate* __restrict__ gates,
                       int n_gates, const double2* __restrict__ bsk, const double2* __restrict__ tw_g,
                       const double2* __restrict__ psi_g, const uint16_t* __restrict__ leaf_g,
                       uint64_t* __restrict__ arena, int slot_stride, const uint64_t* __restrict__ sel) {
    fbr_rotate<N, K, E, LAT, B, false, true>(ks, ks_stride, n, gates, n_gates, bsk, tw_g, psi_g, leaf_g, arena,
                                             slot_stride, nullptr, sel);
}

template <int N>
__global__ void __launch_bounds__(N / 8)
k_key_products(const uint64_t* __restrict__ ks, int ks_stride, int n, int n_gates, const double2* __restrict__ bsk,
               const double2* __restrict__ psi_g, double2* __restrict__ kpre) {
    constexpr int K = 1, E = 4, M = N / 2, T = M / E;
    using G = FGeo<M, E>;
    static_assert(G::key_slot_matches_idx(), "the Fourier key's lane layout is the last-phase layout");
    constexpr int LAST = G::NPH - 1, LOG2N2 = G::LOG + 2;
    constexpr uint32_t GG = (uint32_t)(K + 1) * (K + 1) * M;
    __shared__ __attribute__((aligned(16))) double2 psi[N / 2];
    const int tl = threadIdx.x, t = (int)blockIdx.x, P = (int)blockIdx.y;
    const int steps = (n + 1) / 2;
    for (int i = tl; i < N / 2; i += T) psi[psi_slot(i)] = psi_g[i];
    const __amdgpu_buffer_rsrc_t rs = bsk_rsrc(bsk);
    const uint32_t lane_off = 16u * (uint32_t)tl, sb = (uint32_t)t * (3u * GG * 16u);
    double2 gv[3][K + 1][E];
#pragma unroll
    for (int gg = 0; gg < 3; ++gg)
#pragma unroll
        for (int m = 0; m < E; ++m) {
            gv[gg][0][m] = bsk_load(rs, lane_off, sb + 16u * (gg * GG + (uint32_t)(P * (K + 1) + P) * M + (uint32_t)m * T));
            gv[gg][1][m] = bsk_load(
                rs, lane_off, sb + 16u * (gg * GG + (uint32_t)(other_row<K>(P, 0) * (K + 1) + P) * M + (uint32_t)m * T));
        }
    const uint32_t Lb = (1u + 4u * (__brev((uint32_t)G::template idx<LAST>(tl, 0)) >> (32 - G::LOG))) & (uint32_t)(M - 1);
    __syncthreads();
    for (int b = 0; b < n_gates; ++b) {
        const uint64_t* in = ks + (size_t)b * ks_stride;
        const uint32_t ei = (uint16_t)mod_switch(in[2 * t], LOG2N2);
        const uint32_t ej = 2 * t + 1 < n ? (uint16_t)mod_switch(in[2 * t + 1], LOG2N2) : 0u;
        if ((ei | ej) == 0) continue;
        double br[2][1], bi[2][1];
        key_psi_base<N, true>(psi, ei, Lb, br[0][0], bi[0][0]);
        key_psi_base<N, true>(psi, ej, Lb, br[1][0], bi[1][0]);
        double2* out = kpre + (((size_t)b * steps + t) * (K + 1) + P) * ((K + 1) * M) + tl;
#pragma unroll
        for (int m = 0; m < E; ++m) {
            const uint32_t sm = ((m & 1) << 1) | ((m >> 1) & 1);
            double kor, koi, kxr[K], kxi[K];
            key_products<K>(br, bi, 0, ei, ej, sm, [&](int gg, int r) __attribute__((always_inline)) { return gv[gg][r][m]; },
                            kor, koi, kxr, kxi);
            out[m * T] = make_double2(kor, koi);
            out[(E + m) * T] = make_double2(kxr[0], kxi[0]);
        }
    }
}

#ifndef FR_BR_PAIR_TU
extern template __global__ void k_blind_rotate_fft<2048, 1, 4, true, 2>(const uint64_t*, int, int, const DevGate*, int,
                                                                         const double2*, const double2*, const double2*,
                                                                         const uint16_t*, uint64_t*, int);
extern template __global__ void k_blind_rotate_fft_acc<2048, 1, 4, true, 2>(const uint64_t*, int, int, const DevGate*,
                                                                             int, const double2*, const double2*,
                                                                             const double2*, const uint16_t*, uint64_t*,
                                                                             int, const uint64_t*);
#endif

template <int N>
constexpr size_t fbr_dual_smem_bytes() {
    return 16 * (2 * (size_t)FGeo<N / 2, 4>::NP + (size_t)N / 2) + 16 * MAX_OUT + 2 * 1026 + 4 * 16 * MAX_OUT +
           4 * MAX_OUT;
}
template <int N>
__global__ void __launch_bounds__(N / 8, 2)
k_blind_rotate_fft_dual(const uint64_t* __restrict__ ks, int ks_stride, int n, const DevGate* __restrict__ gates,
                        int n_gates, const double2* __restrict__ bsk, const double2* __restrict__ tw_g,
                        const double2* __restrict__ psi_g, const uint16_t* __restrict__ leaf_g,
                        uint64_t* __restrict__ arena, int slot_stride) {
    constexpr int K = 1, E = 4, M = N / 2, B = 2;
    using G = FGeo<M, E>;
    static_assert(fexchanges_conflict_free<M, E>(), "LDS maps must make every exchange conflict-free");
    static_assert(G::base_matches_geo(), "base<p> must be the index map the LDS-map proofs reason about");
    static_assert(G::key_slot_matches_idx(), "the Fourier key's lane layout is the last-phase layout");
    static_assert(fradix4<M, E>(), "dual shape: the k = 1 geometry (radix-4 inverse)");
    constexpr int T = M / E, NT = T, LAST = G::NPH - 1;
    constexpr int LOG2N2 = G::LOG + 2;
    constexpr int BS = G::NP;
    extern __shared__ __attribute__((aligned(16))) double2 fsm[];
    double2* xbuf = fsm;
    double2* psi = xbuf + B * BS;
    uint8_t* lut = (uint8_t*)(psi + N / 2);
    uint16_t* abar = (uint16_t*)(lut + 16 * MAX_OUT);
    uint32_t* wterms = (uint32_t*)(abar + 1026);
    int* wcnt = (int*)(wterms + 16 * MAX_OUT);

    const int tl = threadIdx.x;
    const int gi = (int)blockIdx.x;
    const uint64_t* in = ks + (size_t)gi * ks_stride;
    const int n_out = gates[gi].n_out, kind = gates[gi].direct;
    for (int i = tl; i < N / 2; i += NT) psi[psi_slot(i)] = psi_g[i];
    for (int i = tl; i < 16 * n_out; i += NT) lut[i] = gates[gi].lut[i / 16][i % 16];
    for (int i = tl; i < n; i += NT) abar[i] = (uint16_t)mod_switch(in[i], LOG2N2);
    if (tl == 0) abar[n] = 0;
    const uint32_t bbar = mod_switch(in[n], LOG2N2);
    const uint32_t Lb = (1u + 4u * (__brev((uint32_t)G::template idx<LAST>(tl, 0)) >> (32 - G::LOG))) & (uint32_t)(M - 1);
    __syncthreads();

    double alo[B][E], ahi[B][E];
    {
        const bool direct = kind == JOB_DIRECT;
#pragma unroll
        for (int m = 0; m < E; ++m) {
            const int j = G::template idx<0>(tl, m);
            uint64_t v[2];
#pragma unroll
            for (int h = 0; h < 2; ++h) {
                const int s = (j + h * M + (int)bbar) & (2 * N - 1);
                const uint64_t tv = test_poly<N>(s & (N - 1), direct, lut);
                v[h] = s < N ? tv : (uint64_t)0 - tv;
            }
#pragma unroll
            for (int P = 0; P < B; ++P) {
                alo[P][m] = P == K ? fft::acc_of_torus(v[0]) : 0.0;
                ahi[P][m] = P == K ? fft::acc_of_torus(v[1]) : 0.0;
            }
        }
    }
    constexpr uint32_t GG = (uint32_t)(K + 1) * (K + 1) * M;
    const __amdgpu_buffer_rsrc_t rs = bsk_rsrc(bsk);
    const uint32_t lane_off = 16u * (uint32_t)tl;
    const int steps = (n + 1) / 2;
    FTwr<M, E> twr;
    ftw_load_phase<M, E, 0, FR_TW_SGPR_PAIR>(twr, tw_g, tl);
    auto load_keys = [&](double2 (&Bk)[3][2][2], uint32_t sbase, int m) {
#pragma unroll
        for (int gg = 0; gg < 3; ++gg)
#pragma unroll
            for (int r = 0; r < 2; ++r)
#pragma unroll
                for (int c = 0; c < 2; ++c)
                    Bk[gg][r][c] =
                        bsk_load(rs, lane_off, sbase + 16u * (gg * GG + (uint32_t)(r * 2 + c) * M + (uint32_t)m * T));
    };
    for (int t = 0; t < steps; ++t) {
        if ((abar[2 * t] | abar[2 * t + 1]) == 0) continue;
        const uint32_t sbase = (uint32_t)__builtin_amdgcn_readfirstlane(t) * (3u * GG * 16u);
        double2 Bc[3][2][2];
        load_keys(Bc, sbase, 0);
        const uint32_t ei = __builtin_amdgcn_readfirstlane((uint32_t)abar[2 * t]);
        const uint32_t ej = __builtin_amdgcn_readfirstlane((uint32_t)abar[2 * t + 1]);
        double2 x[B][E];
#pragma unroll
        for (int P = 0; P < B; ++P)
#pragma unroll
            for (int m = 0; m < E; ++m)
                x[P][m] = make_double2(fft::acc_digit<23>(alo[P][m]), fft::acc_digit<23>(ahi[P][m]));
        fforward_from<M, E, 0, false, true, B, BS>(x, xbuf, twr, nullptr, tl, [](auto) {});
        double bre[2], bim[2];
#pragma unroll
        for (int h = 0; h < 2; ++h) {
            const uint32_t k = __umul24(h == 0 ? ei : ej, Lb) & (2 * N - 1);
            const double2 q = psi[psi_slot((int)(k & (N / 2 - 1)))];
            fft::psi_quadrant(q.x, q.y, k >> (LOG2N2 - 2), bre[h], bim[h]);
        }
#pragma unroll
        for (int m = 0; m < E; ++m) {
            double2 Bn[3][2][2];
            if (m + 1 < E) load_keys(Bn, sbase, m + 1);
            __builtin_amdgcn_sched_barrier(0);
            const uint32_t sm = ((m & 1) << 1) | ((m >> 1) & 1);
            double cr[3], ci[3];
#pragma unroll
            for (int h = 1; h < 3; ++h) slot_factor(bre[h - 1], bim[h - 1], h == 1 ? ei : ej, sm, cr[h], ci[h]);
            fft::cmul(cr[1], ci[1], cr[2], ci[2], cr[0], ci[0]);
            double2 z[B];
#pragma unroll
            for (int c = 0; c < B; ++c) {
                double kor, koi, kxr, kxi;
#pragma unroll
                for (int gg = 0; gg < 3; ++gg) {
                    const double c1r = cr[gg] - 1.0, c1i = ci[gg];
                    const double2 Bo = Bc[gg][c][c], Bx = Bc[gg][1 - c][c];
                    if (gg == 0) {
                        fft::cmul(Bo.x, Bo.y, c1r, c1i, kor, koi);
                        fft::cmul(Bx.x, Bx.y, c1r, c1i, kxr, kxi);
                    } else {
                        fft::cmac(Bo.x, Bo.y, c1r, c1i, kor, koi);
                        fft::cmac(Bx.x, Bx.y, c1r, c1i, kxr, kxi);
                    }
                }
                double zr, zi;
                fft::cmul(x[c][m].x, x[c][m].y, kor, koi, zr, zi);
                fft::cmac(x[1 - c][m].x, x[1 - c][m].y, kxr, kxi, zr, zi);
                z[c] = make_double2(zr, zi);
            }
#pragma unroll
            for (int c = 0; c < B; ++c) x[c][m] = z[c];
            __builtin_amdgcn_sched_barrier(0);
            if (m + 1 < E) {
#pragma unroll
                for (int gg = 0; gg < 3; ++gg)
#pragma unroll
                    for (int r = 0; r < 2; ++r)
#pragma unroll
                        for (int c = 0; c < 2; ++c) Bc[gg][r][c] = Bn[gg][r][c];
            }
        }
        finverse_from<M, E, LAST, false, true, B, BS>(x, xbuf, twr, nullptr, nullptr, tl);
#pragma unroll
        for (int P = 0; P < B; ++P)
#pragma unroll
            for (int m = 0; m < E; ++m) {
                alo[P][m] = fft::acc_reduce<23>(alo[P][m] + x[P][m].x);
                ahi[P][m] = fft::acc_reduce<23>(ahi[P][m] + x[P][m].y);
            }
    }

    __syncthreads();
    uint64_t* accs = (uint64_t*)xbuf;
    static_assert(8 * B * N <= 16 * B * BS, "dual shape: u64 rows inside the exchange rows");
#pragma unroll
    for (int P = 0; P < B; ++P) fbr_publish<M, E>(accs + P * N, alo[P], ahi[P], tl);
    fbr_terms<N>(tl, n_out, kind, lut, wterms, wcnt);
    __syncthreads();
    if (gi >= n_gates) return;
    fbr_outputs<N, K, NT>(tl, accs, gates[gi], n_out, kind, wterms, wcnt, arena, slot_stride);
}

#ifndef FR_BR_PAIR_TU
constexpr bool fft_supported(int K, int N, int E) {
    return (K == 1 && N == 2048 && E == 4) || (K == 2 && N == 1024 && (E == 4 || E == 8));
}

template <int N, int K, int E, bool LAT, int B = 1>
static void fft_attr() {
    static_assert(fbr_smem_bytes<N, K, E, LAT, B>() <= (LAT ? 160 * 1024 : 160 * 1024 / fbr_tp_groups<K, E>()),
                  "LDS per workgroup of the shape");
    HIP_CHECK(hipFuncSetAttribute((const void*)k_blind_rotate_fft<N, K, E, LAT, B>,
                                  hipFuncAttributeMaxDynamicSharedMemorySize, (int)fbr_smem_bytes<N, K, E, LAT, B>()));
    HIP_CHECK(hipFuncSetAttribute((const void*)k_blind_rotate_fft_acc<N, K, E, LAT, B>,
                                  hipFuncAttributeMaxDynamicSharedMemorySize, (int)fbr_smem_bytes<N, K, E, LAT, B>()));
}

template <class F>
static void fft_dispatch(const Params& p, F&& body) {
    if (p.k == 1 && p.N == 2048) body(std::integral_constant<int, 2048>{}, std::integral_constant<int, 1>{});
    else if (p.k == 2 && p.N == 1024) body(std::integral_constant<int, 1024>{}, std::integral_constant<int, 2>{});
    else throw Error(FR_ERR_INVALID, "device: FFT ring needs (k, N) in {(1, 2048), (2, 1024)}");
}

void Device::init_fft() {
    if (p_.k == 2) fft_e_ = 8;
    if (const char* ev = std::getenv("FR_FFT_LANE_ELEMS")) fft_e_ = std::atoi(ev);
    if (const char* ev = std::getenv("FR_FFT_SMALL_BATCH")) fft_small_ = (size_t)std::atol(ev);
    if (const char* ev = std::getenv("FR_FFT_PAIR_BATCH")) fft_pair_ = (size_t)std::atol(ev);
    if (const char* ev = std::getenv("FR_FFT_DUAL")) fft_dual_ = std::atoi(ev) != 0;
    if (const char* ev = std::getenv("FR_FFT_KPRE_BATCH")) fft_kpre_ = (size_t)std::atol(ev);
    if (p_.k != 1) fft_pair_ = 0, fft_kpre_ = 0;
    if (!fft_supported(p_.k, p_.N, fft_e_))
        throw Error(FR_ERR_INVALID, "device: FFT ring needs (k, N, E) in {(1, 2048, 4), (2, 1024, 4 or 8)}");
    fft_dispatch(p_, [&](auto nc, auto kc) {
        constexpr int N = decltype(nc)::value, K = decltype(kc)::value;
        fft_attr<N, K, 4, true>();
        fft_attr<N, K, 4, false>();
        if constexpr (K == 1) {
            fft_attr<N, K, 4, true, 2>();
            static_assert(fbr_smem_bytes<N, K, 4, true, 1, true>() <= 160 * 1024, "LDS per workgroup of the shape");
            HIP_CHECK(hipFuncSetAttribute((const void*)k_blind_rotate_fft_kp<N, K, 4, true, 1>,
                                          hipFuncAttributeMaxDynamicSharedMemorySize,
                                          (int)fbr_smem_bytes<N, K, 4, true, 1, true>()));
            static_assert(fbr_dual_smem_bytes<N>() <= 80 * 1024, "dual shape: two workgroups per CU");
            HIP_CHECK(hipFuncSetAttribute((const void*)k_blind_rotate_fft_dual<N>,
                                          hipFuncAttributeMaxDynamicSharedMemorySize, (int)fbr_dual_smem_bytes<N>()));
        }
        if constexpr (fft_supported(K, N, 8)) fft_attr<N, K, 8, false>();
    });

    fft::Tables T(p_.N);
    d_ftw_.alloc(2 * (size_t)T.M);
    std::vector<fft::c64> psi(2 * (size_t)p_.N);
    for (int k = 0; k < 2 * p_.N; ++k) psi[k] = fft::psi_pow(p_.N, k);
    d_fqt_.alloc(2 * psi.size());
    d_fleaf_.alloc((size_t)T.M);
    HIP_CHECK(hipMemcpy(d_ftw_.get(), T.tw.data(), 16 * (size_t)T.M, hipMemcpyHostToDevice));
    HIP_CHECK(hipMemcpy(d_fqt_.get(), psi.data(), 16 * psi.size(), hipMemcpyHostToDevice));
    HIP_CHECK(hipMemcpy(d_fleaf_.get(), T.leaf.data(), 2 * (size_t)T.M, hipMemcpyHostToDevice));
}

void Device::upload_fft_bsk(const std::vector<uint64_t>& bsk) {
    const int N = p_.N, M = N / 2, kp1 = p_.k + 1;
    const size_t polys = p_.bsk_ggsw() * (size_t)kp1 * kp1;
    fft::Tables tabs(N);
    std::vector<fft::c64> four;
    fft::bsk_to_fourier(tabs, bsk, polys, four);
    std::vector<fft::c64> lanes(four.size());
    for (int E : {8, 4}) {
        gpu::DevBuf<double>& dst = d_fbsk_[fbsk_index(E)];
        dst.reset();
        if (!fft_supported(p_.k, N, E) || !fbsk_needed(E)) continue;
        const int T = M / E, e = ilog2c(E);
        std::vector<int> slot((size_t)M);
        for (int q = 0; q < M; ++q) slot[q] = fft_key_slot(tabs.LOG, e, q % T, q / T);
        for (size_t pq = 0; pq < polys; ++pq)
            for (size_t q = 0; q < (size_t)M; ++q) lanes[pq * M + q] = four[pq * M + slot[q]];
        dst.alloc(2 * lanes.size());
        HIP_CHECK(hipMemcpy(dst.get(), lanes.data(), 16 * lanes.size(), hipMemcpyHostToDevice));
    }
}

void Device::launch_br_fft(const DevGate* d_gates, const uint64_t* d_ks, size_t n, hipStream_t s, hipEvent_t ev_start,
                           hipEvent_t ev_stop, bool acc) {
    const uint64_t* sel = cur().sel;
    if (acc && !sel) throw Error(FR_ERR_INVALID, "selector jobs: no selector table bound");
    auto launch = [&](auto kernel, size_t grid, int threads, size_t lds, int E, auto... more) {
        hipExtLaunchKernelGGL(kernel, dim3((unsigned)grid), dim3(threads), (uint32_t)lds, s, ev_start, ev_stop, 0, d_ks,
                              p_.ks_stride(), p_.n, d_gates, (int)n, (const double2*)d_fbsk_[fbsk_index(E)].get(),
                              (const double2*)d_ftw_.get(), (const double2*)d_fqt_.get(),
                              (const uint16_t*)d_fleaf_.get(), d_arena_.get(), p_.slot_stride(), more...);
    };
    fft_dispatch(p_, [&](auto nc, auto kc) {
        constexpr int N = decltype(nc)::value, K = decltype(kc)::value;
        auto go = [&](auto ec, auto lat, auto bc) {
            constexpr int E = decltype(ec)::value;
            constexpr bool LAT = decltype(lat)::value;
            constexpr int B = decltype(bc)::value;
            if constexpr (fft_supported(K, N, E) && (B == 1 || K == 1)) {
                if (acc)
                    launch(k_blind_rotate_fft_acc<N, K, E, LAT, B>, (n + B - 1) / B, fbr_threads<N, K, E>(),
                           fbr_smem_bytes<N, K, E, LAT, B>(), E, sel);
                else
                    launch(k_blind_rotate_fft<N, K, E, LAT, B>, (n + B - 1) / B, fbr_threads<N, K, E>(),
                           fbr_smem_bytes<N, K, E, LAT, B>(), E);
            }
        };
        using I4 = std::integral_constant<int, 4>;
        using I8 = std::integral_constant<int, 8>;
        using B1 = std::integral_constant<int, 1>;
        if (n <= fft_small_ && n <= fft_kpre_ && K == 1 && !acc) {
            if constexpr (K == 1) {
                const int steps = (p_.n + 1) / 2;
                const size_t per = (size_t)steps * (kpre_step_bytes<N, K>() / 8);
                gpu::DevBuf<double>& kpre = cur().kpre;
                if (kpre.size() < n * per) {
                    HIP_CHECK(hipStreamSynchronize(s));
                    kpre.alloc(n * per);
                }
                hipExtLaunchKernelGGL(k_key_products<N>, dim3((unsigned)steps, K + 1), dim3(N / 8), 0, s, ev_start,
                                      nullptr, 0, d_ks, p_.ks_stride(), p_.n, (int)n,
                                      (const double2*)d_fbsk_[fbsk_index(4)].get(), (const double2*)d_fqt_.get(),
                                      (double2*)kpre.get());
                hipExtLaunchKernelGGL((k_blind_rotate_fft_kp<N, K, 4, true, 1>), dim3((unsigned)n),
                                      dim3(fbr_threads<N, K, 4>()), (uint32_t)fbr_smem_bytes<N, K, 4, true, 1, true>(), s,
                                      nullptr, ev_stop, 0, d_ks, p_.ks_stride(), p_.n, d_gates, (int)n,
                                      (const double2*)d_ftw_.get(), d_arena_.get(), p_.slot_stride(),
                                      (const double2*)kpre.get());
            }
        } else if (n <= fft_small_) go(I4{}, std::true_type{}, B1{});
        else if (n <= fft_pair_ && K == 1 && fft_dual_ && !acc) {
            if constexpr (K == 1) launch(k_blind_rotate_fft_dual<N>, n, N / 8, fbr_dual_smem_bytes<N>(), 4);
        } else if (n <= fft_pair_) go(I4{}, std::true_type{}, std::integral_constant<int, 2>{});
        else if (fft_e_ == 4) go(I4{}, std::false_type{}, B1{});
        else go(I8{}, std::false_type{}, B1{});
    });
    HIP_CHECK(hipGetLastError());
}

#endif

}
```

Measured before the change: 127,600.

## Split key-product blind rotation to overlap precompute with rotation on aux stream

For small latency batches, the precomputed key-products blind rotation is split at a step boundary. The front steps' key products are computed first. The remaining steps' products are then produced on an auxiliary stream while the first rotation segment runs, and the accumulators are saved to global memory and resumed. The key-products rotation moves to a dedicated kernel in its own translation unit, with an option to fetch products one or two steps ahead. This trades extra accumulator traffic, an extra launch and more stream and event management for hiding the precompute latency.

```diff
diff --git a/fhe-regex_amd/csrc/device.h b/fhe-regex_amd/csrc/device.h
--- a/fhe-regex_amd/csrc/device.h
+++ b/fhe-regex_amd/csrc/device.h
@@ -134,6 +134,9 @@
         gpu::DevBuf<uint64_t> pk_g;
         gpu::DevBuf<uint16_t> pk_c16;
         gpu::DevBuf<double> kpre;
+        gpu::DevBuf<double> kacc;
+        gpu::Stream aux;
+        gpu::Event front_ev, aux_ev;
         gpu::StagingRing<int> cmap;
         size_t cmap_n = 0;
         const uint64_t* sel = nullptr;
@@ -176,8 +179,8 @@
     void build_limbs(LimbKey& key);
     void drop_server_key() {
         ksk_.reset(), d_tbsk_.reset(), d_bsk_.reset(), d_fbsk_[0].reset(), d_fbsk_[1].reset();
-        lane0_.kpre.reset();
-        for (auto& l : lanes_) l.kpre.reset();
+        lane0_.kpre.reset(), lane0_.kacc.reset();
+        for (auto& l : lanes_) l.kpre.reset(), l.kacc.reset();
     }
     void drop_packing_key() { pksk_.reset(); }
     struct KsShape {
@@ -243,6 +246,9 @@
     size_t fft_pair_ = SIZE_MAX;
     bool fft_dual_ = false;
     size_t fft_kpre_ = 32;
+    int fft_kpre_ahead_ = 1;
+    size_t fft_kpre_split_ = 8;
+    int kp_split_steps(size_t n) const;
     gpu::DevBuf<double> d_fbsk_[2];
     static int fbsk_index(int E) { return E == 4 ? 0 : 1; }
     bool fbsk_needed(int E) const { return E == 4 || E == fft_e_; }
diff --git a/fhe-regex_amd/csrc/device.hip b/fhe-regex_amd/csrc/device.hip
--- a/fhe-regex_amd/csrc/device.hip
+++ b/fhe-regex_amd/csrc/device.hip
@@ -90,6 +90,9 @@
     (void)hipSetDevice(dev_);
     for (auto& l : lanes_) (void)hipStreamSynchronize(l.stream.get());
     if (lane0_.stream) (void)hipStreamSynchronize(lane0_.stream.get());
+    for (auto& l : lanes_)
+        if (l.aux) (void)hipStreamSynchronize(l.aux.get());
+    if (lane0_.aux) (void)hipStreamSynchronize(lane0_.aux.get());
 }
 
 void Device::set_lanes(int n) {
@@ -142,6 +145,9 @@
 void Device::sync_all() {
     HIP_CHECK(hipStreamSynchronize(lane0_.stream.get()));
     for (auto& l : lanes_) HIP_CHECK(hipStreamSynchronize(l.stream.get()));
+    if (lane0_.aux) HIP_CHECK(hipStreamSynchronize(lane0_.aux.get()));
+    for (auto& l : lanes_)
+        if (l.aux) HIP_CHECK(hipStreamSynchronize(l.aux.get()));
     if (lane_ == 0) {
         for (auto& l : lanes_) l.pending = false;
         lanes_pending_ = false;
diff --git a/fhe-regex_amd/csrc/fft_br.hip b/fhe-regex_amd/csrc/fft_br.hip
--- a/fhe-regex_amd/csrc/fft_br.hip
+++ b/fhe-regex_amd/csrc/fft_br.hip
@@ -6,6 +6,10 @@
 #include "device_impl.h"
 #include "fft.h"
 #include "geo.h"
+
+#if defined(FR_BR_PAIR_TU) || defined(FR_BR_KP_TU)
+#define FR_BR_KERNELS_ONLY 1
+#endif
 
 namespace fr {
 
@@ -506,14 +510,12 @@
     return 16u * (uint32_t)((K + 1) * (K + 1) * (N / 2));
 }
 
-template <int N, int K, int E, bool LAT, int B, bool KP, bool ACC = false>
+template <int N, int K, int E, bool LAT, int B, bool ACC = false>
 __device__ __forceinline__ void fbr_rotate(const uint64_t* ks, int ks_stride, int n, const DevGate* gates, int n_gates,
                                            const double2* bsk, const double2* tw_g, const double2* psi_g,
-                                           const uint16_t* leaf_g, uint64_t* arena, int slot_stride, const double2* kpre,
+                                           const uint16_t* leaf_g, uint64_t* arena, int slot_stride,
                                            const uint64_t* sel = nullptr) {
     constexpr int M = N / 2;
-    static_assert(!KP || (LAT && B == 1 && K == 1 && E == 4), "key products: the k = 1 latency shape");
-    static_assert(!(ACC && KP), "selector launches never take the key-products path");
     using G = FGeo<M, E>;
     static_assert(fexchanges_conflict_free<M, E>(), "LDS maps must make every exchange conflict-free");
     static_assert(G::base_matches_geo(), "base<p> must be the index map the LDS-map proofs reason about");
@@ -530,7 +532,7 @@
     double2* xbuf = fsm;
     double2* ibuf = LAT ? xbuf + B * BS : xbuf;
     double2* tw = xbuf + (LAT ? 2 : 1) * B * BS;
-    constexpr int NPSI = KP ? 0 : PSIQ ? N / 2 : 2 * N;
+    constexpr int NPSI = PSIQ ? N / 2 : 2 * N;
     double2* psi = tw + (B == 1 ? M : 0);
     double2* twc = psi + NPSI;
     constexpr int NTWC = fbr_twc_entries<N, K, E, LAT>();
@@ -627,8 +629,7 @@
     const __amdgpu_buffer_rsrc_t rs = bsk_rsrc(bsk);
     const uint32_t lane_off = 16u * (uint32_t)tl;
     const int steps = (n + 1) / 2;
-    double2 gv[3][K + 1][LAT && !KP ? E : 1];
-    double2 kv[K + 1][KP ? E : 1];
+    double2 gv[3][K + 1][LAT ? E : 1];
     FTwr<M, TWR ? E : 2> twr;
     if constexpr (TWR) ftw_load_phase<M, E, 0, B == 1 ? false : FR_TW_SGPR_PAIR>(twr, B == 1 ? tw : tw_g, tl);
 #ifdef FR_BR_TIMING
@@ -637,33 +638,19 @@
     const uint64_t tstart = tlast;
 #endif
     auto load_ggsw = [&](int gg, int tt) {
-        if constexpr (!KP) {
-            const uint32_t sb = (uint32_t)__builtin_amdgcn_readfirstlane(tt) * (3u * GG * 16u);
-#pragma unroll
-            for (int m = 0; m < E; ++m) {
-                gv[gg][0][m] =
-                    bsk_load(rs, lane_off, sb + 16u * (gg * GG + (uint32_t)(P * (K + 1) + P) * M + (uint32_t)m * T));
-#pragma unroll
-                for (int q = 0; q < K; ++q)
-                    gv[gg][1 + q][m] = bsk_load(
-                        rs, lane_off,
-                        sb + 16u * (gg * GG + (uint32_t)(other_row<K>(P, q) * (K + 1) + P) * M + (uint32_t)m * T));
-            }
+        const uint32_t sb = (uint32_t)__builtin_amdgcn_readfirstlane(tt) * (3u * GG * 16u);
+#pragma unroll
+        for (int m = 0; m < E; ++m) {
+            gv[gg][0][m] =
+                bsk_load(rs, lane_off, sb + 16u * (gg * GG + (uint32_t)(P * (K + 1) + P) * M + (uint32_t)m * T));
+#pragma unroll
+            for (int q = 0; q < K; ++q)
+                gv[gg][1 + q][m] = bsk_load(
+                    rs, lane_off,
+                    sb + 16u * (gg * GG + (uint32_t)(other_row<K>(P, q) * (K + 1) + P) * M + (uint32_t)m * T));
         }
     };
-    const __amdgpu_buffer_rsrc_t rk =
-        bsk_rsrc(KP ? kpre + (size_t)blockIdx.x * ((size_t)((n + 1) / 2) * (kpre_step_bytes<N, K>() / 16)) : bsk);
-    auto load_kp = [&](int tt) {
-        if constexpr (KP) {
-            const uint32_t sb = (uint32_t)__builtin_amdgcn_readfirstlane(tt) * kpre_step_bytes<N, K>();
-#pragma unroll
-            for (int r = 0; r <= K; ++r)
-#pragma unroll
-                for (int m = 0; m < E; ++m)
-                    kv[r][m] = bsk_load(rk, lane_off, sb + 16u * (uint32_t)(((P * (K + 1) + r) * E + m) * T));
-        }
-    };
-    constexpr int NPF = KP ? 0 : LAT ? (B > 1 ? FR_PAIR_PF : K == 1 ? FR_LAT_PF : FR_LAT_PF2) : 0;
+    constexpr int NPF = LAT ? (B > 1 ? FR_PAIR_PF : K == 1 ? FR_LAT_PF : FR_LAT_PF2) : 0;
     constexpr bool LATPF = NPF > 0;
     auto idle = [&](int t) {
         uint32_t z = 0;
@@ -671,7 +658,7 @@
         for (int b = 0; b < B; ++b) z |= abar[b * 1026 + 2 * t] | abar[b * 1026 + 2 * t + 1];
         return z == 0;
     };
-    if constexpr (LATPF || KP) {
+    if constexpr (LATPF) {
         for (int t = tid; t <= steps; t += NT) {
             int tt = t;
             while (tt < steps && idle(tt)) ++tt;
@@ -680,15 +667,14 @@
         __syncthreads();
         const int t0 = __builtin_amdgcn_readfirstlane((int)nxt[0]);
         for (int gg = 0; gg < NPF; ++gg) load_ggsw(gg, t0 < steps ? t0 : 0);
-        load_kp(t0 < steps ? t0 : 0);
     }
     for (int t = 0; t < steps; ++t) {
         if (idle(t)) continue;
         BR_STAMP(0);
         const uint32_t sbase = (uint32_t)__builtin_amdgcn_readfirstlane(t) * (3u * GG * 16u);
-        constexpr int G_TOP = !LAT || KP || B > 1 ? 3 : (NPF < 2 || K == 1) ? NPF : 3;
-        constexpr int G_L1 = !LAT || KP ? 3 : B > 1 ? NPF : G_TOP + 1 < 3 ? G_TOP + 1 : 3;
-        constexpr int G_L2 = !LAT || KP ? 3 : B > 1 ? (NPF + 1 < 3 ? NPF + 1 : 3) : G_TOP == 3 ? NPF : G_TOP + 2 < 3 ? G_TOP + 2 : 3;
+        constexpr int G_TOP = !LAT || B > 1 ? 3 : (NPF < 2 || K == 1) ? NPF : 3;
+        constexpr int G_L1 = !LAT ? 3 : B > 1 ? NPF : G_TOP + 1 < 3 ? G_TOP + 1 : 3;
+        constexpr int G_L2 = !LAT ? 3 : B > 1 ? (NPF + 1 < 3 ? NPF + 1 : 3) : G_TOP == 3 ? NPF : G_TOP + 2 < 3 ? G_TOP + 2 : 3;
         constexpr int PH_L1 = B > 1 ? FR_PAIR_LOAD : FR_LAT_LOAD1;
         constexpr int PH_L2 = B > 1 ? FR_PAIR_LOAD2 : FR_LAT_LOAD2;
         static_assert(G_L1 >= 3 || PH_L1 < G::NPH, "FR_PAIR_LOAD / FR_LAT_LOAD1 past the last forward phase");
@@ -714,7 +700,7 @@
                     for (int bb = 0; bb < NB; ++bb)
                         key_psi_base<N, PSIQ>(psi, h == 0 ? ei[b] : ej[b], Lb[bb], bre[b][h][bb], bim[b][h][bb]);
         };
-        if constexpr (LAT && B == 1 && !KP) psi_factors();
+        if constexpr (LAT && B == 1) psi_factors();
         double2 x[B][E];
 #pragma unroll
         for (int b = 0; b < B; ++b)
@@ -764,17 +750,11 @@
 #pragma unroll
                 for (int q = 0; q < K; ++q) oth[q] = orow_bl[q][b * BS + G::template at<XL>(G::template moff<LAST>(m))];
                 double kor, koi, kxr[K], kxi[K];
-                if constexpr (KP) {
-                    kor = kv[0][m].x, koi = kv[0][m].y;
-#pragma unroll
-                    for (int q = 0; q < K; ++q) kxr[q] = kv[1 + q][m].x, kxi[q] = kv[1 + q][m].y;
-                } else {
-                    const uint32_t sm = ((m & 1) << 1) | ((m >> 1) & 1);
-                    auto key_at = [&](int gg, int r) __attribute__((always_inline)) {
-                        return LAT ? gv[gg][r][LAT ? m : 0] : Bc[gg][r];
-                    };
-                    key_products<K>(bre[b], bim[b], m >> 2, ei[b], ej[b], sm, key_at, kor, koi, kxr, kxi);
-                }
+                const uint32_t sm = ((m & 1) << 1) | ((m >> 1) & 1);
+                auto key_at = [&](int gg, int r) __attribute__((always_inline)) {
+                    return LAT ? gv[gg][r][LAT ? m : 0] : Bc[gg][r];
+                };
+                key_products<K>(bre[b], bim[b], m >> 2, ei[b], ej[b], sm, key_at, kor, koi, kxr, kxi);
                 double zr, zi;
                 fft::cmul(own.x, own.y, kor, koi, zr, zi);
 #pragma unroll
@@ -791,11 +771,10 @@
                     for (int r = 0; r <= K; ++r) Bc[gg][r] = Bn[gg][r];
             }
         }
-        if constexpr (LATPF || KP) {
+        if constexpr (LATPF) {
             const int tn = __builtin_amdgcn_readfirstlane((int)nxt[t + 1]);
             __builtin_amdgcn_sched_barrier(0);
             for (int gg = 0; gg < NPF; ++gg) load_ggsw(gg, tn < steps ? tn : t);
-            load_kp(tn < steps ? tn : t);
             __builtin_amdgcn_sched_barrier(0);
         }
         BR_STAMP(3);
@@ -840,39 +819,29 @@
                    int n_gates, const double2* __restrict__ bsk, const double2* __restrict__ tw_g,
                    const double2* __restrict__ psi_g, const uint16_t* __restrict__ leaf_g, uint64_t* __restrict__ arena,
                    int slot_stride) {
-    fbr_rotate<N, K, E, LAT, B, false>(ks, ks_stride, n, gates, n_gates, bsk, tw_g, psi_g, leaf_g, arena, slot_stride,
-                                       nullptr);
-}
-template <int N, int K, int E, bool LAT, int B = 1>
-__global__ void __launch_bounds__((fbr_threads<N, K, E>()), (fbr_min_waves<N, K, E, LAT>()))
-k_blind_rotate_fft_kp(const uint64_t* __restrict__ ks, int ks_stride, int n, const DevGate* __restrict__ gates,
-                      int n_gates, const double2* __restrict__ tw_g, uint64_t* __restrict__ arena, int slot_stride,
-                      const double2* __restrict__ kpre) {
-    fbr_rotate<N, K, E, LAT, B, true>(ks, ks_stride, n, gates, n_gates, nullptr, tw_g, nullptr, nullptr, arena,
-                                      slot_stride, kpre);
-}
-
+    fbr_rotate<N, K, E, LAT, B>(ks, ks_stride, n, gates, n_gates, bsk, tw_g, psi_g, leaf_g, arena, slot_stride);
+}
 template <int N, int K, int E, bool LAT, int B = 1>
 __global__ void __launch_bounds__((fbr_threads<N, K, E>()), (fbr_min_waves<N, K, E, LAT>()))
 k_blind_rotate_fft_acc(const uint64_t* __restrict__ ks, int ks_stride, int n, const DevGate* __restrict__ gates,
                        int n_gates, const double2* __restrict__ bsk, const double2* __restrict__ tw_g,
                        const double2* __restrict__ psi_g, const uint16_t* __restrict__ leaf_g,
                        uint64_t* __restrict__ arena, int slot_stride, const uint64_t* __restrict__ sel) {
-    fbr_rotate<N, K, E, LAT, B, false, true>(ks, ks_stride, n, gates, n_gates, bsk, tw_g, psi_g, leaf_g, arena,
-                                             slot_stride, nullptr, sel);
+    fbr_rotate<N, K, E, LAT, B, true>(ks, ks_stride, n, gates, n_gates, bsk, tw_g, psi_g, leaf_g, arena, slot_stride,
+                                      sel);
 }
 
 template <int N>
 __global__ void __launch_bounds__(N / 8)
 k_key_products(const uint64_t* __restrict__ ks, int ks_stride, int n, int n_gates, const double2* __restrict__ bsk,
-               const double2* __restrict__ psi_g, double2* __restrict__ kpre) {
+               const double2* __restrict__ psi_g, double2* __restrict__ kpre, int t_off) {
     constexpr int K = 1, E = 4, M = N / 2, T = M / E;
     using G = FGeo<M, E>;
     static_assert(G::key_slot_matches_idx(), "the Fourier key's lane layout is the last-phase layout");
     constexpr int LAST = G::NPH - 1, LOG2N2 = G::LOG + 2;
     constexpr uint32_t GG = (uint32_t)(K + 1) * (K + 1) * M;
     __shared__ __attribute__((aligned(16))) double2 psi[N / 2];
-    const int tl = threadIdx.x, t = (int)blockIdx.x, P = (int)blockIdx.y;
+    const int tl = threadIdx.x, t = t_off + (int)blockIdx.x, P = (int)blockIdx.y;
     const int steps = (n + 1) / 2;
     for (int i = tl; i < N / 2; i += T) psi[psi_slot(i)] = psi_g[i];
     const __amdgpu_buffer_rsrc_t rs = bsk_rsrc(bsk);
@@ -888,7 +857,7 @@
         }
     const uint32_t Lb = (1u + 4u * (__brev((uint32_t)G::template idx<LAST>(tl, 0)) >> (32 - G::LOG))) & (uint32_t)(M - 1);
     __syncthreads();
-    for (int b = 0; b < n_gates; ++b) {
+    for (int b = (int)blockIdx.z; b < n_gates; b += (int)gridDim.z) {
         const uint64_t* in = ks + (size_t)b * ks_stride;
         const uint32_t ei = (uint16_t)mod_switch(in[2 * t], LOG2N2);
         const uint32_t ej = 2 * t + 1 < n ? (uint16_t)mod_switch(in[2 * t + 1], LOG2N2) : 0u;
@@ -908,6 +877,213 @@
         }
     }
 }
+
+template <int N>
+constexpr size_t kp_alone_lds() {
+    return 160 * 1024 - 4 * (size_t)N;
+}
+
+template <int N>
+constexpr size_t kp_acc_bytes() {
+    return 8 * 2 * (size_t)N;
+}
+
+template <int N, int AH>
+__device__ __forceinline__ void fbr_rotate_kp(const uint64_t* ks, int ks_stride, int n, const DevGate* gates,
+                                              const double2* tw_g, uint64_t* arena, int slot_stride,
+                                              const double2* kpre, int t_begin, int t_end, double* accs_g) {
+    constexpr int K = 1, E = 4, M = N / 2;
+    static_assert(AH == 1 || AH == 2, "products one or two unskipped steps ahead");
+    static_assert(fbr_twr<K, true>(), "the key-products variant keeps the lane's twiddles in registers");
+    using G = FGeo<M, E>;
+    static_assert(fexchanges_conflict_free<M, E>(), "LDS maps must make every exchange conflict-free");
+    static_assert(G::base_matches_geo(), "base<p> must be the index map the LDS-map proofs reason about");
+    static_assert(G::key_slot_matches_idx(), "the products' lane layout is the last-phase layout");
+    constexpr int T = M / E, NT = (K + 1) * T, LAST = G::NPH - 1, XL = G::XL;
+    constexpr int LOG2N2 = G::LOG + 2;
+    constexpr int BS = (K + 1) * G::NP;
+    extern __shared__ __attribute__((aligned(16))) double2 fsm[];
+    double2* xbuf = fsm;
+    double2* ibuf = xbuf + BS;
+    double2* tw = ibuf + BS;
+    uint8_t* lut = (uint8_t*)(tw + M);
+    uint16_t* abar = (uint16_t*)(lut + 16 * MAX_OUT);
+    uint32_t* wterms = (uint32_t*)(abar + 1026);
+    int* wcnt = (int*)(wterms + 16 * MAX_OUT);
+    uint16_t* nxt = (uint16_t*)(wcnt + MAX_OUT);
+
+    const int tid = threadIdx.x;
+    const int P = __builtin_amdgcn_readfirstlane(tid / T), tl = tid % T;
+    const int gi = (int)blockIdx.x;
+    const uint64_t* in = ks + (size_t)gi * ks_stride;
+    const int n_out = gates[gi].n_out, kind = gates[gi].direct;
+    const int steps = (n + 1) / 2;
+    const bool resume = t_begin > 0, last = t_end >= steps;
+    for (int i = tid; i < M; i += NT) tw[i] = tw_g[i];
+    for (int i = tid; i < 16 * n_out; i += NT) lut[i] = gates[gi].lut[i / 16][i % 16];
+    for (int i = tid; i < n; i += NT) abar[i] = (uint16_t)mod_switch(in[i], LOG2N2);
+    if (tid == 0) abar[n] = 0;
+    const uint32_t bbar = mod_switch(in[n], LOG2N2);
+    __syncthreads();
+
+    double alo[1][E], ahi[1][E];
+    double* acc_t = accs_g + (size_t)gi * (kp_acc_bytes<N>() / 8) + tid;
+    if (resume) {
+#pragma unroll
+        for (int m = 0; m < E; ++m) {
+            alo[0][m] = acc_t[m * NT];
+            ahi[0][m] = acc_t[(E + m) * NT];
+        }
+    } else {
+        const bool direct = kind == JOB_DIRECT;
+#pragma unroll
+        for (int m = 0; m < E; ++m) {
+            const int j = G::template idx<0>(tl, m);
+            uint64_t v[2];
+#pragma unroll
+            for (int h = 0; h < 2; ++h) {
+                const int s = (j + h * M + (int)bbar) & (2 * N - 1);
+                const uint64_t tv = test_poly<N>(s & (N - 1), direct, lut);
+                v[h] = s < N ? tv : (uint64_t)0 - tv;
+            }
+            alo[0][m] = P == K ? fft::acc_of_torus(v[0]) : 0.0;
+            ahi[0][m] = P == K ? fft::acc_of_torus(v[1]) : 0.0;
+        }
+    }
+
+    double2* row = xbuf + P * G::NP;
+    double2* irow = ibuf + P * G::NP;
+    const int bl = G::template base<LAST>(tl);
+    double2* row_bl = row + G::template at<XL>(bl);
+    const double2* orow_bl = xbuf + other_row<K>(P, 0) * G::NP + G::template at<XL>(bl);
+    const uint32_t lane_off = 16u * (uint32_t)tl;
+    double2 kv[AH][K + 1][E];
+    FTwr<M, E> twr;
+    ftw_load_phase<M, E, 0, false>(twr, tw, tl);
+#ifdef FR_BR_TIMING
+    uint64_t tseg[6] = {0, 0, 0, 0, 0, 0};
+    uint64_t tlast = __builtin_amdgcn_s_memtime();
+    const uint64_t tstart = tlast;
+#endif
+    const __amdgpu_buffer_rsrc_t rk = bsk_rsrc(kpre + (size_t)gi * ((size_t)steps * (kpre_step_bytes<N, K>() / 16)));
+    auto load_kp = [&](auto rc, int tt) {
+        constexpr int R = decltype(rc)::value;
+        const uint32_t sb = (uint32_t)__builtin_amdgcn_readfirstlane(tt) * kpre_step_bytes<N, K>();
+#pragma unroll
+        for (int r = 0; r <= K; ++r)
+#pragma unroll
+            for (int m = 0; m < E; ++m)
+                kv[R][r][m] = bsk_load(rk, lane_off, sb + 16u * (uint32_t)(((P * (K + 1) + r) * E + m) * T));
+    };
+    int mine = 0;
+    for (int t = t_begin + tid; t <= t_end; t += NT) {
+        int tt = t;
+        while (tt < t_end && (abar[2 * tt] | abar[2 * tt + 1]) == 0) ++tt;
+        nxt[t] = (uint16_t)tt;
+        mine += tt == t && t < t_end;
+    }
+#pragma unroll
+    for (int d = 32; d > 0; d >>= 1) mine += __shfl_xor(mine, d);
+    if ((tid & 63) == 0) wterms[tid >> 6] = (uint32_t)mine;
+    __syncthreads();
+    int live = 0;
+    for (int w = 0; w < NT / 64; ++w) live += (int)wterms[w];
+    live = __builtin_amdgcn_readfirstlane(live);
+    auto next_of = [&](int t) { return __builtin_amdgcn_readfirstlane((int)nxt[t < t_end ? t + 1 : t_end]); };
+    const int t0 = __builtin_amdgcn_readfirstlane((int)nxt[t_begin]);
+    const int t1 = next_of(t0);
+    __builtin_amdgcn_sched_barrier(0);
+    load_kp(std::integral_constant<int, 0>{}, t0 < t_end ? t0 : t_begin);
+    __builtin_amdgcn_sched_barrier(0);
+    if constexpr (AH == 2) load_kp(std::integral_constant<int, 1>{}, t1 < t_end ? t1 : t_begin);
+    __builtin_amdgcn_sched_barrier(0);
+    auto step = [&](int t, auto rc) __attribute__((always_inline)) {
+        constexpr int R = decltype(rc)::value;
+        BR_STAMP(0);
+        double2 x[1][E];
+#pragma unroll
+        for (int m = 0; m < E; ++m) x[0][m] = make_double2(fft::acc_digit<23>(alo[0][m]), fft::acc_digit<23>(ahi[0][m]));
+        BR_STAMP(1);
+        fforward_from<M, E, 0, true, true, 1, BS>(x, row, twr, tw, tl, [](auto) {});
+        BR_STAMP(2);
+#pragma unroll
+        for (int m = 0; m < E; ++m) row_bl[G::template at<XL>(G::template moff<LAST>(m))] = x[0][m];
+        __syncthreads();
+#pragma unroll
+        for (int m = 0; m < E; ++m) {
+            const double2 own = x[0][m];
+            const double2 oth = orow_bl[G::template at<XL>(G::template moff<LAST>(m))];
+            double zr, zi;
+            fft::cmul(own.x, own.y, kv[R][0][m].x, kv[R][0][m].y, zr, zi);
+            fft::cmac(oth.x, oth.y, kv[R][1][m].x, kv[R][1][m].y, zr, zi);
+            x[0][m] = make_double2(zr, zi);
+        }
+        {
+            int ta = next_of(t);
+            if constexpr (AH == 2) ta = next_of(ta);
+            __builtin_amdgcn_sched_barrier(0);
+            load_kp(rc, ta < t_end ? ta : t);
+            __builtin_amdgcn_sched_barrier(0);
+        }
+        BR_STAMP(3);
+        finverse_from<M, E, LAST, true, true, 1, BS>(x, irow, twr, tw, nullptr, tl);
+        BR_STAMP(4);
+#pragma unroll
+        for (int m = 0; m < E; ++m) {
+            alo[0][m] = fft::acc_reduce<23>(alo[0][m] + x[0][m].x);
+            ahi[0][m] = fft::acc_reduce<23>(ahi[0][m] + x[0][m].y);
+        }
+        BR_STAMP(5);
+    };
+    int t = t0;
+    for (int i = 0; i < live / AH; ++i) {
+        step(t, std::integral_constant<int, 0>{});
+        t = next_of(t);
+        if constexpr (AH == 2) {
+            step(t, std::integral_constant<int, 1>{});
+            t = next_of(t);
+        }
+    }
+    if (AH == 2 && (live & 1)) step(t, std::integral_constant<int, 0>{});
+#ifdef FR_BR_TIMING
+    if (blockIdx.x == 0 && tid == 0)
+        printf("FBR_TIMING E=%d LAT=%d steps=%d total=%lu digits=%lu fwd=%lu mac=%lu inv=%lu acc=%lu top=%lu\n", E, 1,
+               t_end - t_begin, (unsigned long)(__builtin_amdgcn_s_memtime() - tstart), (unsigned long)tseg[1],
+               (unsigned long)tseg[2], (unsigned long)tseg[3], (unsigned long)tseg[4], (unsigned long)tseg[5],
+               (unsigned long)tseg[0]);
+#endif
+    if (!last) {
+#pragma unroll
+        for (int m = 0; m < E; ++m) {
+            acc_t[m * NT] = alo[0][m];
+            acc_t[(E + m) * NT] = ahi[0][m];
+        }
+        return;
+    }
+    __syncthreads();
+    uint64_t* accs = (uint64_t*)xbuf;
+    fbr_publish<M, E>(accs + P * N, alo[0], ahi[0], tl);
+    fbr_terms<N>(tid, n_out, kind, lut, wterms, wcnt);
+    __syncthreads();
+    fbr_outputs<N, K, NT>(tid, accs, gates[gi], n_out, kind, wterms, wcnt, arena, slot_stride);
+}
+
+template <int N, int K, int E, bool LAT, int B = 1, int AH = 1>
+__global__ void __launch_bounds__((fbr_threads<N, K, E>()), (fbr_min_waves<N, K, E, LAT>()))
+k_blind_rotate_fft_kp(const uint64_t* __restrict__ ks, int ks_stride, int n, const DevGate* __restrict__ gates,
+                      const double2* __restrict__ tw_g, uint64_t* __restrict__ arena, int slot_stride,
+                      const double2* __restrict__ kpre, int t_begin, int t_end, double* __restrict__ accs) {
+    static_assert(K == 1 && E == 4 && LAT && B == 1, "key products: the k = 1 latency shape");
+    fbr_rotate_kp<N, AH>(ks, ks_stride, n, gates, tw_g, arena, slot_stride, kpre, t_begin, t_end, accs);
+}
+#ifndef FR_BR_KP_TU
+extern template __global__ void k_blind_rotate_fft_kp<2048, 1, 4, true, 1, 1>(const uint64_t*, int, int, const DevGate*,
+                                                                               const double2*, uint64_t*, int,
+                                                                               const double2*, int, int, double*);
+extern template __global__ void k_blind_rotate_fft_kp<2048, 1, 4, true, 1, 2>(const uint64_t*, int, int, const DevGate*,
+                                                                               const double2*, uint64_t*, int,
+                                                                               const double2*, int, int, double*);
+#endif
 
 #ifndef FR_BR_PAIR_TU
 extern template __global__ void k_blind_rotate_fft<2048, 1, 4, true, 2>(const uint64_t*, int, int, const DevGate*, int,
@@ -1080,7 +1256,7 @@
     fbr_outputs<N, K, NT>(tl, accs, gates[gi], n_out, kind, wterms, wcnt, arena, slot_stride);
 }
 
-#ifndef FR_BR_PAIR_TU
+#ifndef FR_BR_KERNELS_ONLY
 constexpr bool fft_supported(int K, int N, int E) {
     return (K == 1 && N == 2048 && E == 4) || (K == 2 && N == 1024 && (E == 4 || E == 8));
 }
@@ -1109,6 +1285,9 @@
     if (const char* ev = std::getenv("FR_FFT_PAIR_BATCH")) fft_pair_ = (size_t)std::atol(ev);
     if (const char* ev = std::getenv("FR_FFT_DUAL")) fft_dual_ = std::atoi(ev) != 0;
     if (const char* ev = std::getenv("FR_FFT_KPRE_BATCH")) fft_kpre_ = (size_t)std::atol(ev);
+    if (const char* ev = std::getenv("FR_FFT_KPRE_AHEAD")) fft_kpre_ahead_ = std::atoi(ev);
+    if (const char* ev = std::getenv("FR_FFT_KPRE_SPLIT")) fft_kpre_split_ = (size_t)std::atol(ev);
+    if (fft_kpre_ahead_ != 1 && fft_kpre_ahead_ != 2) throw Error(FR_ERR_INVALID, "device: FR_FFT_KPRE_AHEAD is 1 or 2");
     if (p_.k != 1) fft_pair_ = 0, fft_kpre_ = 0;
     if (!fft_supported(p_.k, p_.N, fft_e_))
         throw Error(FR_ERR_INVALID, "device: FFT ring needs (k, N, E) in {(1, 2048, 4), (2, 1024, 4 or 8)}");
@@ -1119,9 +1298,11 @@
         if constexpr (K == 1) {
             fft_attr<N, K, 4, true, 2>();
             static_assert(fbr_smem_bytes<N, K, 4, true, 1, true>() <= 160 * 1024, "LDS per workgroup of the shape");
-            HIP_CHECK(hipFuncSetAttribute((const void*)k_blind_rotate_fft_kp<N, K, 4, true, 1>,
-                                          hipFuncAttributeMaxDynamicSharedMemorySize,
-                                          (int)fbr_smem_bytes<N, K, 4, true, 1, true>()));
+            static_assert(fbr_smem_bytes<N, K, 4, true, 1, true>() <= kp_alone_lds<N>(), "LDS of a rotation alone on its CU");
+            HIP_CHECK(hipFuncSetAttribute((const void*)k_blind_rotate_fft_kp<N, K, 4, true, 1, 1>,
+                                          hipFuncAttributeMaxDynamicSharedMemorySize, (int)kp_alone_lds<N>()));
+            HIP_CHECK(hipFuncSetAttribute((const void*)k_blind_rotate_fft_kp<N, K, 4, true, 1, 2>,
+                                          hipFuncAttributeMaxDynamicSharedMemorySize, (int)kp_alone_lds<N>()));
             static_assert(fbr_dual_smem_bytes<N>() <= 80 * 1024, "dual shape: two workgroups per CU");
             HIP_CHECK(hipFuncSetAttribute((const void*)k_blind_rotate_fft_dual<N>,
                                           hipFuncAttributeMaxDynamicSharedMemorySize, (int)fbr_dual_smem_bytes<N>()));
@@ -1159,6 +1340,13 @@
         dst.alloc(2 * lanes.size());
         HIP_CHECK(hipMemcpy(dst.get(), lanes.data(), 16 * lanes.size(), hipMemcpyHostToDevice));
     }
+}
+
+int Device::kp_split_steps(size_t n) const {
+    if (!fft_kpre_split_ || n < fft_kpre_split_) return 0;
+    const int steps = (p_.n + 1) / 2;
+    const int s0 = (int)((42 * n + 26 * 8 - 1) / (26 * 8)) * 8;
+    return s0 + 8 <= steps ? s0 : 0;
 }
 
 void Device::launch_br_fft(const DevGate* d_gates, const uint64_t* d_ks, size_t n, hipStream_t s, hipEvent_t ev_start,
@@ -1193,20 +1381,49 @@
             if constexpr (K == 1) {
                 const int steps = (p_.n + 1) / 2;
                 const size_t per = (size_t)steps * (kpre_step_bytes<N, K>() / 8);
-                gpu::DevBuf<double>& kpre = cur().kpre;
-                if (kpre.size() < n * per) {
+                LaneState& l = cur();
+                const int s0 = kp_split_steps(n);
+                if (l.kpre.size() < n * per || (s0 && l.kacc.size() < n * (kp_acc_bytes<N>() / 8))) {
                     HIP_CHECK(hipStreamSynchronize(s));
-                    kpre.alloc(n * per);
+                    if (l.aux) HIP_CHECK(hipStreamSynchronize(l.aux.get()));
+                    if (l.kpre.size() < n * per) l.kpre.alloc(n * per);
+                    if (s0 && l.kacc.size() < n * (kp_acc_bytes<N>() / 8)) l.kacc.alloc(n * (kp_acc_bytes<N>() / 8));
                 }
-                hipExtLaunchKernelGGL(k_key_products<N>, dim3((unsigned)steps, K + 1), dim3(N / 8), 0, s, ev_start,
-                                      nullptr, 0, d_ks, p_.ks_stride(), p_.n, (int)n,
-                                      (const double2*)d_fbsk_[fbsk_index(4)].get(), (const double2*)d_fqt_.get(),
-                                      (double2*)kpre.get());
-                hipExtLaunchKernelGGL((k_blind_rotate_fft_kp<N, K, 4, true, 1>), dim3((unsigned)n),
-                                      dim3(fbr_threads<N, K, 4>()), (uint32_t)fbr_smem_bytes<N, K, 4, true, 1, true>(), s,
-                                      nullptr, ev_stop, 0, d_ks, p_.ks_stride(), p_.n, d_gates, (int)n,
-                                      (const double2*)d_ftw_.get(), d_arena_.get(), p_.slot_stride(),
-                                      (const double2*)kpre.get());
+                auto produce = [&](hipStream_t q, int t0, int t1, size_t nz, hipEvent_t e0) {
+                    hipExtLaunchKernelGGL(k_key_products<N>, dim3((unsigned)(t1 - t0), K + 1, (unsigned)nz),
+                                          dim3(N / 8), 0, q, e0, nullptr, 0, d_ks, p_.ks_stride(), p_.n, (int)n,
+                                          (const double2*)d_fbsk_[fbsk_index(4)].get(), (const double2*)d_fqt_.get(),
+                                          (double2*)l.kpre.get(), t0);
+                };
+                auto rotate = [&](int t0, int t1, hipEvent_t e1, size_t lds = fbr_smem_bytes<N, K, 4, true, 1, true>()) {
+                    auto go_kp = [&](auto kernel) {
+                        hipExtLaunchKernelGGL(kernel, dim3((unsigned)n), dim3(fbr_threads<N, K, 4>()),
+                                              (uint32_t)lds, s, nullptr, e1, 0, d_ks,
+                                              p_.ks_stride(), p_.n, d_gates, (const double2*)d_ftw_.get(),
+                                              d_arena_.get(), p_.slot_stride(), (const double2*)l.kpre.get(), t0, t1,
+                                              l.kacc.get());
+                    };
+                    if (fft_kpre_ahead_ == 2) go_kp(k_blind_rotate_fft_kp<N, K, 4, true, 1, 2>);
+                    else go_kp(k_blind_rotate_fft_kp<N, K, 4, true, 1, 1>);
+                };
+                if (!s0) {
+                    produce(s, 0, steps, 1, ev_start);
+                    rotate(0, steps, ev_stop);
+                } else {
+                    if (!l.aux) {
+                        l.aux.create();
+                        l.front_ev = take_event();
+                        l.aux_ev = take_event();
+                    }
+                    produce(s, 0, s0, n, ev_start);
+                    HIP_CHECK(hipEventRecord(l.front_ev.get(), s));
+                    HIP_CHECK(hipStreamWaitEvent(l.aux.get(), l.front_ev.get(), 0));
+                    produce(l.aux.get(), s0, steps, 1, nullptr);
+                    HIP_CHECK(hipEventRecord(l.aux_ev.get(), l.aux.get()));
+                    rotate(0, s0, nullptr, kp_alone_lds<N>());
+                    HIP_CHECK(hipStreamWaitEvent(s, l.aux_ev.get(), 0));
+                    rotate(s0, steps, ev_stop);
+                }
             }
         } else if (n <= fft_small_) go(I4{}, std::true_type{}, B1{});
         else if (n <= fft_pair_ && K == 1 && fft_dual_ && !acc) {
diff --git a/fhe-regex_amd/csrc/fft_br_kp.hip b/fhe-regex_amd/csrc/fft_br_kp.hip
--- /dev/null
+++ b/fhe-regex_amd/csrc/fft_br_kp.hip
@@ -0,0 +1,11 @@
+#define FR_BR_KP_TU 1
+#include "fft_br.hip"
+
+namespace fr {
+template __global__ void k_blind_rotate_fft_kp<2048, 1, 4, true, 1, 1>(const uint64_t*, int, int, const DevGate*,
+                                                                        const double2*, uint64_t*, int, const double2*,
+                                                                        int, int, double*);
+template __global__ void k_blind_rotate_fft_kp<2048, 1, 4, true, 1, 2>(const uint64_t*, int, int, const DevGate*,
+                                                                        const double2*, uint64_t*, int, const double2*,
+                                                                        int, int, double*);
+}
```

Result: no change. 127,700 (median of 3 runs) (+0.0%).
